# Litianyu141/Gen-FVGN-steady

Hardware: AMD Instinct MI355X
Metric: training iters/sec, 50k-cell cylinder mesh (fwd + loss + bwd + Adam, batch resident in HBM) (higher is better)
Workload: dtype f32

## Files before the change

### gen-fvgn-steady_amd/csrc/colchain.hip

```cpp
#include "colchain_kernel.h"

int* gfv_internal_status_ptr();

static int cc_env(const char* name, int dflt) {
  const char* e = getenv(name);
  return e ? atoi(e) : dflt;
}
static bool al16(const void* p) { return (reinterpret_cast<size_t>(p) & 15) == 0; }

static int cc_cus() {
  static int n = 0;
  if (!n) {
    int dev = 0;
    hipDeviceProp_t pr;
    if (hipGetDevice(&dev) == hipSuccess && hipGetDeviceProperties(&pr, dev) == hipSuccess) n = pr.multiProcessorCount;
    if (n <= 0) n = 256;
    const int want = cc_env("GFV_COLCHAIN_WGS", 0);
    if (want > 0 && want <= n) n = want;
  }
  return n;
}

static bool cc_bwd_ok(const gfv_rowtile_args_t* a) {
  static const int on = cc_env("GFV_COLCHAIN_BWD", 1);
  static const int min_m = cc_env("GFV_COLCHAIN_BWD_MIN_M", 2048);
  if (a->flags & GFV_CHAIN_ROW_OWNER) return false;
  if (!(a->flags & GFV_CHAIN_COLUMN_OWNER) && (!on || a->M < min_m)) return false;
  if (!a->dw_partial || a->dw_partial_stride < GFV_DW_FUSED_FLOATS || !a->in_stats || !a->wmax) return false;
  if (a->dw_in) return false;
  const bool noout = a->nlayers == 2;
  const bool rc = a->rc_Wh[0] != nullptr;
  if (rc && (!a->rc_Wh[1] || a->dw_in || !al16(a->rc_Wh[0]) || !al16(a->rc_Wh[1]) || (a->rc_bias[0] && !al16(a->rc_bias[0])) ||
             (a->rc_bias[1] && !al16(a->rc_bias[1]))))
    return false;
  if (!rc && a->rc_Wh[1]) return false;
  if ((a->nlayers != 3 && !noout) || a->in_op != GFV_IN_LNBWD || a->fin_op != GFV_FIN_PLAIN || a->nseg != 1) return false;
  if (noout && (a->layer[1].op != GFV_OP_MUL_DGELU || a->layer[1].save || a->res[0] || a->gadd || a->dw_in || !a->out[0])) return false;
  if (a->seg[0].width != 128 || a->seg[0].idx || a->seg[0].csr_rowptr || a->seg[0].save || a->seg[0].ld != 128 || !al16(a->seg[0].ptr)) return false;
  if (a->M > (1 << 22) || a->out_ld[0] != 128 || (a->res[0] && a->res_ld[0] != 128) || (a->dw_in && a->dw_in_ld != 128)) return false;
  if (a->layer[0].op != GFV_OP_MUL_DGELU || a->layer[1].op != GFV_OP_MUL_DGELU || (!noout && a->layer[2].op != GFV_OP_NONE)) return false;
  for (int l = 0; l < a->nlayers; ++l) {
    const gfv_layer_t& L = a->layer[l];
    if (!L.Wh || (L.N != 128 && !(l == 2 && L.N == 192)) || L.K != 128 || L.bias || L.bias2) return false;
    if (l < 2 && !(rc && l == 0) && (!L.aux || !al16(L.aux))) return false;
    if (L.save && !al16(L.save)) return false;
  }
  if ((!rc && (!a->in_aux || !al16(a->in_aux))) || !a->in_gamma || !al16(a->in_gamma) || a->ln_partial || a->padd) return false;
  const bool out2 = !noout && a->layer[2].N == 192;
  if (!a->out[0] || (out2 ? (!a->out[1] || a->out_ld[1] != 64 || !al16(a->out[1]) || a->dw_in) : a->out[1] != nullptr) || a->out[2] ||
      a->res[1] || a->res[2] || a->out_nores)
    return false;
  if ((a->out_ld[0] & 3) || !al16(a->out[0]) || (a->res[0] && ((a->res_ld[0] & 3) || !al16(a->res[0])))) return false;
  if (a->in_add && !al16(a->in_add)) return false;
  if (a->gadd && (!al16(a->gadd) || !a->gadd_s || !a->gadd_r)) return false;
  if (a->in_save && !al16(a->in_save)) return false;
  if ((reinterpret_cast<size_t>(a->in_stats) & 7) || !al16(a->dw_partial) || (a->dw_partial_stride & 3)) return false;
  return true;
}
extern "C" int gfv_hidden_size(void);
extern "C" int gfv_f16split_enabled(void);
extern "C" int gfv_rowtile_dw_partials(void) { return cc_cus(); }
extern "C" int gfv_rowtile_dw_partials_m(int32_t M) {
  const int tiles = (M + 63) / 64;
  return tiles < cc_cus() ? (tiles > 0 ? tiles : 1) : cc_cus();
}
extern "C" int gfv_rowtile_fuses_dw(const gfv_rowtile_args_t* a) {
  if (!a || gfv_hidden_size() != 128 || gfv_f16split_enabled() == 0) return 0;
  gfv_rowtile_args_t t = *a;
  t.hidden = 128;
  return cc_bwd_ok(&t) ? 1 : 0;
}

int gfv_internal_colchain_try(const gfv_rowtile_args_t* a, hipStream_t stream) {
  if (a->hidden == 128 && cc_bwd_ok(a)) {
    int* st = gfv_internal_status_ptr();
    if (!st) return 0;
    const dim3 grid(gfv_rowtile_dw_partials_m(a->M)), blk(64 * CC_W);
#define CB_K(...) GFV_LAUNCH((colchain_bwd_kernel<__VA_ARGS__>), grid, blk, 0, stream, *a, st)
#define CB_LAUNCH(LOWP, RC)                                                                                                      \
  do {                                                                                                                           \
    if (a->nlayers == 2) CB_K(LOWP, false, false, true, RC);                                                                     \
    else if (a->layer[2].N == 192 && a->gadd) CB_K(LOWP, true, true, false, RC);                                                 \
    else if (a->layer[2].N == 192) CB_K(LOWP, false, true, false, RC);                                                           \
    else if (a->gadd) CB_K(LOWP, true, false, false, RC);                                                                        \
    else CB_K(LOWP, false, false, false, RC);                                                                                    \
  } while (0)
    const bool rc = a->rc_Wh[0] != nullptr;
    if (a->product_form == 2) { if (rc) CB_LAUNCH(2, true); else CB_LAUNCH(2, false); }
    else if (a->product_form != 0) { if (rc) CB_LAUNCH(1, true); else CB_LAUNCH(1, false); }
    else { if (rc) CB_LAUNCH(0, true); else CB_LAUNCH(0, false); }
#undef CB_K
#undef CB_LAUNCH
    return 2;
  }
  return 0;
}
```

### gen-fvgn-steady_amd/csrc/colchain_kernel.h

```cpp
#pragma once
#include "tchain_kernel.h"

namespace {

constexpr int CC_W = 8;
constexpr float CC_SH = 16.0f;
constexpr float CC_SH_INV = 1.0f / 16.0f;
constexpr float CC_SH_LIMIT = 2048.0f;
#ifdef GFV_CC_TIMING
#define CT_DECL long long ct_[16] = {0, 0, 0, 0, 0, 0, 0, 0, 0, 0, 0, 0, 0, 0, 0, 0}; long long ct_prev_ = clock64();
#define CT(k) do { __builtin_amdgcn_s_waitcnt(0xc07f); const long long now_ = clock64(); ct_[k] += now_ - ct_prev_; ct_prev_ = now_; } while (0)
#else
#define CT_DECL
#define CT(k)
#endif
__device__ __forceinline__ void cc_barrier() {
  asm volatile("s_waitcnt lgkmcnt(0)\n\ts_barrier" ::: "memory");
}

struct CcCtx {
  int w, lane, j, g, col0;
  int M;
  int row0;
  int ngt;
  float invw;
  float mabs;
};

template <int KT, int LOWP, bool FENCE = false>
__device__ __forceinline__ void cc_mma_pair(const char* xbuf, int pair, const gfv_f16x8 (&wh)[KT], const gfv_f16x8 (&wl)[KT],
                                            int lane, floatx4& a0, floatx4& a1) {
  const gfv_f16x8* f0 = reinterpret_cast<const gfv_f16x8*>(xbuf + (size_t)(2 * pair) * KT * 2048) + lane;
  const gfv_f16x8* f1 = f0 + KT * 128;
  a0 = floatx4{0.f, 0.f, 0.f, 0.f};
  a1 = floatx4{0.f, 0.f, 0.f, 0.f};
#pragma unroll
  for (int T = 0; T < KT; ++T) {
    const gfv_f16x8 xh0 = f0[(2 * T) * 64], xh1 = f1[(2 * T) * 64];
    if (!LOWP) {
      const gfv_f16x8 xl0 = f0[(2 * T + 1) * 64], xl1 = f1[(2 * T + 1) * 64];
      a0 = __builtin_amdgcn_mfma_f32_16x16x32_f16(wl[T], xh0, a0, 0, 0, 0);
      a1 = __builtin_amdgcn_mfma_f32_16x16x32_f16(wl[T], xh1, a1, 0, 0, 0);
      a0 = __builtin_amdgcn_mfma_f32_16x16x32_f16(wh[T], xl0, a0, 0, 0, 0);
      a1 = __builtin_amdgcn_mfma_f32_16x16x32_f16(wh[T], xl1, a1, 0, 0, 0);
    }
    a0 = gfv_mma_hh<LOWP == 2>(wh[T], xh0, a0);
    a1 = gfv_mma_hh<LOWP == 2>(wh[T], xh1, a1);
    if (FENCE) __builtin_amdgcn_sched_barrier(0);
  }
}

template <bool BF>
__device__ __forceinline__ void cc_put_frag(char* xbuf, int q, const CcCtx& c, const float (&a)[4], float scale) {
  unsigned h0, h1, l0, l1;
  const gfv_f2 s01 = gfv_f2{a[0], a[1]} * gfv_splat2(scale), s23 = gfv_f2{a[2], a[3]} * gfv_splat2(scale);
  gfv_split_pair_t<BF>(s01.x, s01.y, h0, l0);
  gfv_split_pair_t<BF>(s23.x, s23.y, h1, l1);
  char* dst = xbuf + (size_t)((q * 4 + (c.w >> 1)) * 2) * 1024 + c.lane * 16 + (c.w & 1) * 8;
  *reinterpret_cast<uint2*>(dst) = make_uint2(h0, h1);
  *reinterpret_cast<uint2*>(dst + 1024) = make_uint2(l0, l1);
}

constexpr int CB_TG = 4;
struct CbLds {
  static constexpr int BUF = CB_TG * 8192;
  static constexpr int B0 = 0, B1 = BUF, B2 = 2 * BUF;
  static constexpr int PART = 3 * BUF;
  static constexpr int SMAX = PART + CB_TG * 16 * 8 * 8;
  static constexpr int TOTAL = SMAX + 64;
};

__device__ __forceinline__ void cb_tr_operand(const char* xbuf, int q0, int ct, int lane, gfv_f16x8& hi, gfv_f16x8& lo) {
  typedef short s4 __attribute__((ext_vector_type(4)));
  typedef __attribute__((address_space(3))) s4* lds_s4;
  const int s = lane & 15, gp = lane >> 4;
  const int off = ((q0 * 4 + (ct >> 1)) * 2) * 1024 + (16 * (s & 3) + 4 * gp + (s >> 2)) * 16 + (ct & 1) * 8;
  const char* p = xbuf + off;
  const s4 h0 = __builtin_amdgcn_ds_read_tr16_b64_v4i16((lds_s4)(p));
  const s4 l0 = __builtin_amdgcn_ds_read_tr16_b64_v4i16((lds_s4)(p + 1024));
  const s4 h1 = __builtin_amdgcn_ds_read_tr16_b64_v4i16((lds_s4)(p + 8192));
  const s4 l1 = __builtin_amdgcn_ds_read_tr16_b64_v4i16((lds_s4)(p + 8192 + 1024));
  typedef short s8 __attribute__((ext_vector_type(8)));
  const s8 h = {h0[0], h0[1], h0[2], h0[3], h1[0], h1[1], h1[2], h1[3]};
  const s8 l = {l0[0], l0[1], l0[2], l0[3], l1[0], l1[1], l1[2], l1[3]};
  hi = __builtin_bit_cast(gfv_f16x8, h);
  lo = __builtin_bit_cast(gfv_f16x8, l);
}

__device__ __forceinline__ int cb_dw_ntile(int w, int i) { return 2 * (w >> 1) + (i >> 2); }
__device__ __forceinline__ int cb_dw_ktile(int w, int i) { return 4 * (w & 1) + (i & 3); }
__device__ __forceinline__ int cb_dw_btile(int w) { return 2 * (w >> 1) + (w & 1); }
template <int LOWP>
__device__ __forceinline__ void cb_dw_tile(const char* gbuf, const char* abuf, int npairs, int w, int lane, floatx4 (&acc)[8],
                                           floatx4& accb) {
  const gfv_f16x8 ones = gfv_frag_ones<LOWP == 2>();
  const int nt0 = 2 * (w >> 1), kt0 = 4 * (w & 1);
  for (int pr = 0; pr < npairs; ++pr) {
    gfv_f16x8 gh[2], gl[2];
    cb_tr_operand(gbuf, 2 * pr, nt0, lane, gh[0], gl[0]);
    cb_tr_operand(gbuf, 2 * pr, nt0 + 1, lane, gh[1], gl[1]);
    {
      const bool odd = (w & 1) != 0;
      const gfv_f16x8 bh = odd ? gh[1] : gh[0], bl = odd ? gl[1] : gl[0];
      if (!LOWP) accb = __builtin_amdgcn_mfma_f32_16x16x32_f16(bl, ones, accb, 0, 0, 0);
      accb = gfv_mma_hh<LOWP == 2>(bh, ones, accb);
    }
#pragma unroll
    for (int kk = 0; kk < 4; ++kk) {
      gfv_f16x8 ah, al;
      cb_tr_operand(abuf, 2 * pr, kt0 + kk, lane, ah, al);
#pragma unroll
      for (int nn = 0; nn < 2; ++nn) {
        if (!LOWP) {
          acc[4 * nn + kk] = __builtin_amdgcn_mfma_f32_16x16x32_f16(gl[nn], ah, acc[4 * nn + kk], 0, 0, 0);
          acc[4 * nn + kk] = __builtin_amdgcn_mfma_f32_16x16x32_f16(gh[nn], al, acc[4 * nn + kk], 0, 0, 0);
        }
        acc[4 * nn + kk] = gfv_mma_hh<LOWP == 2>(gh[nn], ah, acc[4 * nn + kk]);
      }
    }
    __builtin_amdgcn_sched_barrier(0);
  }
}

template <bool BF>
__device__ __forceinline__ void cb_hidden_bwd(CcCtx& c, int q, const floatx4& acc, float inv_in, const float4& z, float sg,
                                              char* gout, char* aout, float (&v)[4]) {
  const gfv_f2 z01 = {z.x, z.y}, z23 = {z.z, z.w};
  gfv_f2 a01, a23, d01, d23;
  gfv_gelu_dgelu2(z01, a01, d01);
  gfv_gelu_dgelu2(z23, a23, d23);
  const gfv_f2 ki = gfv_splat2(inv_in), kw = gfv_splat2(c.invw);
  const gfv_f2 v01 = ((gfv_f2{acc[0], acc[1]} * ki) * kw) * d01, v23 = ((gfv_f2{acc[2], acc[3]} * ki) * kw) * d23;
  v[0] = v01.x; v[1] = v01.y; v[2] = v23.x; v[3] = v23.y;
  const float a[4] = {a01.x, a01.y, a23.x, a23.y};
  const float mq = max3_abs(max3_abs(0.f, v[0], v[1]), v[2], v[3]) * sg;
  const float ma = max3_abs(max3_abs(0.f, a[0], a[1]), a[2], a[3]) * (60000.0f / CC_SH_LIMIT);
  c.mabs = fmaxf(c.mabs, q < c.ngt ? fmaxf(mq, ma) : 0.f);
  cc_put_frag<BF>(gout, q, c, v, sg);
  cc_put_frag<BF>(aout, q, c, a, CC_SH);
}

__device__ __forceinline__ char* cb_own_slot(char* xbuf, int q, const CcCtx& c) {
  return xbuf + (size_t)((q * 4 + (c.w >> 1)) * 2) * 1024 + c.lane * 16 + (c.w & 1) * 8;
}
__device__ __forceinline__ void cb_park4(char* xbuf, int q, const CcCtx& c, const float (&v)[4]) {
  char* d = cb_own_slot(xbuf, q, c);
  *reinterpret_cast<float2*>(d) = make_float2(v[0], v[1]);
  *reinterpret_cast<float2*>(d + 1024) = make_float2(v[2], v[3]);
}
__device__ __forceinline__ void cb_unpark4(char* xbuf, int q, const CcCtx& c, float (&v)[4]) {
  const char* d = cb_own_slot(xbuf, q, c);
  const float2 a = *reinterpret_cast<const float2*>(d), b = *reinterpret_cast<const float2*>(d + 1024);
  v[0] = a.x; v[1] = a.y; v[2] = b.x; v[3] = b.y;
}

template <bool BF>
__device__ __forceinline__ void cb_hidden_bwd_dg(CcCtx& c, int q, const floatx4& acc, float inv_in, const float (&dg)[4], float sg,
                                                 char* gout, float (&v)[4]) {
#pragma unroll
  for (int r = 0; r < 4; ++r) v[r] = ((acc[r] * inv_in) * c.invw) * dg[r];
  const float mq = max3_abs(max3_abs(0.f, v[0], v[1]), v[2], v[3]) * sg;
  c.mabs = fmaxf(c.mabs, q < c.ngt ? mq : 0.f);
  cc_put_frag<BF>(gout, q, c, v, sg);
}

typedef int cb_i32x4 __attribute__((ext_vector_type(4)));
typedef int cb_i32x2 __attribute__((ext_vector_type(2)));
typedef __amdgpu_buffer_rsrc_t cb_rsrc;
constexpr int CB_OFF_DEAD = 0x7ffffff0;
__device__ __forceinline__ cb_rsrc cb_buf(const void* p, size_t bytes) {
  const size_t n = p ? (bytes < 0x7fffffe0ull ? bytes : 0x7fffffe0ull) : 0;
  return __builtin_amdgcn_make_buffer_rsrc(const_cast<void*>(p), 0, (int)n, 0x00020000);
}
typedef float cb_f32x2 __attribute__((ext_vector_type(2)));
__device__ __forceinline__ float4 cb_ld4(cb_rsrc r, int off) {
  const floatx4 f = __builtin_bit_cast(floatx4, __builtin_amdgcn_raw_buffer_load_b128(r, off, 0, 0));
  return make_float4(f[0], f[1], f[2], f[3]);
}
__device__ __forceinline__ float2 cb_ld2(cb_rsrc r, int off) {
  const cb_f32x2 f = __builtin_bit_cast(cb_f32x2, __builtin_amdgcn_raw_buffer_load_b64(r, off, 0, 0));
  return make_float2(f[0], f[1]);
}
__device__ __forceinline__ void cb_st4v(cb_rsrc r, int off, const floatx4& f) {
  __builtin_amdgcn_raw_buffer_store_b128(__builtin_bit_cast(cb_i32x4, f), r, off, 0, 0);
}
__device__ __forceinline__ void cb_st4(cb_rsrc r, int off, const float (&v)[4]) {
  const floatx4 f = {v[0], v[1], v[2], v[3]};
  __builtin_amdgcn_raw_buffer_store_b128(__builtin_bit_cast(cb_i32x4, f), r, off, 0, 0);
}

struct CbIn {
  float4 dy[CB_TG], yv[CB_TG], ga[CB_TG];
  float2 st[CB_TG];
};
struct CbBufs {
  cb_rsrc dy, y3, stats, z2, z1, gadd, gidx, save1, res, out;
};
__device__ __forceinline__ int cb_off(const CcCtx& c, int row0, int q) { return min(row0 + 16 * q + c.j, c.M - 1) * 512 + c.col0 * 4; }

template <bool GADD>
__device__ __forceinline__ void cb_load_gidx(const CbBufs& B, const CcCtx& c, int row0, int (&gidx)[CB_TG]) {
  if (GADD) {
#pragma unroll
    for (int q = 0; q < CB_TG; ++q) gidx[q] = __builtin_amdgcn_raw_buffer_load_b32(B.gidx, min(row0 + 16 * q + c.j, c.M - 1) * 4, 0, 0);
  }
}
__device__ __forceinline__ void cb_load_inputs(const CbBufs& B, const CcCtx& c, int row0, CbIn& in) {
#pragma unroll
  for (int q = 0; q < CB_TG; ++q) {
    const int off = cb_off(c, row0, q);
    in.dy[q] = cb_ld4(B.dy, off);
    in.yv[q] = cb_ld4(B.y3, off);
    in.st[q] = cb_ld2(B.stats, min(row0 + 16 * q + c.j, c.M - 1) * 8);
  }
}
__device__ __forceinline__ void cb_load_dy_stats(const CbBufs& B, const CcCtx& c, int row0, CbIn& in) {
#pragma unroll
  for (int q = 0; q < CB_TG; ++q) {
    in.dy[q] = cb_ld4(B.dy, cb_off(c, row0, q));
    in.st[q] = cb_ld2(B.stats, min(row0 + 16 * q + c.j, c.M - 1) * 8);
  }
}
__device__ __forceinline__ void cb_load_rows(cb_rsrc r, const CcCtx& c, int row0, float4 (&v)[CB_TG]) {
#pragma unroll
  for (int q = 0; q < CB_TG; ++q) v[q] = cb_ld4(r, cb_off(c, row0, q));
}
template <bool GADD>
__device__ __forceinline__ void cb_load_gathers(const CbBufs& B, const CcCtx& c, const int (&gidx)[CB_TG], CbIn& in) {
  if (GADD) {
#pragma unroll
    for (int q = 0; q < CB_TG; ++q) in.ga[q] = cb_ld4(B.gadd, gidx[q] * 256 + (c.col0 & 63) * 4);
  }
}

template <int LOWP, bool GADD, bool OUT2 = false, bool NOOUT = false, bool RC = false>
__global__ __launch_bounds__(64 * CC_W, 2) void colchain_bwd_kernel(const gfv_rowtile_args_t A, int* status) {
  constexpr int TG = CB_TG;
  __shared__ __attribute__((aligned(16))) char lds[CbLds::TOTAL + (RC ? CbLds::BUF : 0)];
  char* b0 = lds + CbLds::B0;
  char* b1 = lds + CbLds::B1;
  char* b2 = lds + CbLds::B2;
  char* b3 = lds + CbLds::TOTAL;
  float* part = reinterpret_cast<float*>(lds + CbLds::PART);
  float* smax = reinterpret_cast<float*>(lds + CbLds::SMAX);

  CcCtx c;
  c.w = __builtin_amdgcn_readfirstlane(threadIdx.x >> 6);
  c.lane = threadIdx.x & 63;
  c.j = c.lane & 15;
  c.g = c.lane >> 4;
  c.col0 = 16 * c.w + 4 * c.g;
  c.M = A.M;
  c.mabs = 0.f;
  c.invw = 1.0f / gfv_pow2_scale(*A.wmax);

  const int nwg = gridDim.x;
  const int wg = (nwg & 7) == 0 ? (int)(blockIdx.x & 7) * (nwg >> 3) + (int)(blockIdx.x >> 3) : (int)blockIdx.x;
  const int NG = (A.M + 15) >> 4;
  const int g_beg = (int)((long)NG * wg / nwg), g_end = (int)((long)NG * (wg + 1) / nwg);

  const size_t rows128 = (size_t)A.M * 512;
  CbBufs B;
  B.dy = cb_buf(A.seg[0].ptr, rows128);
  B.y3 = cb_buf(RC ? nullptr : A.in_aux, rows128);
  B.stats = cb_buf(A.in_stats, (size_t)A.M * 8);
  B.z2 = cb_buf(RC ? nullptr : A.layer[0].aux, rows128);
  B.z1 = cb_buf(A.layer[1].aux, rows128);
  B.gadd = cb_buf(A.gadd, 0x7fffffe0ull);
  B.gidx = cb_buf(c.w < 4 ? A.gadd_s : A.gadd_r, (size_t)A.M * 4);
  B.save1 = cb_buf(NOOUT ? A.out[0] : A.layer[1].save, rows128);
  B.res = cb_buf(NOOUT ? nullptr : A.res[0], rows128);
  B.out = cb_buf(NOOUT ? nullptr : A.out[0], rows128);
  const cb_rsrc out2 = cb_buf(OUT2 ? A.out[1] : nullptr, (size_t)A.M * 256);

  const cb_rsrc w0 = cb_buf(A.layer[0].Wh, 65536), w1 = cb_buf(A.layer[1].Wh, 65536),
                w2 = cb_buf(NOOUT ? nullptr : A.layer[2].Wh, OUT2 ? 131072 : 65536);
  const cb_rsrc rw2 = cb_buf(RC ? A.rc_Wh[0] : nullptr, 65536), rw3 = cb_buf(RC ? A.rc_Wh[1] : nullptr, 65536);
  const int woff = (c.w * 128 + c.lane) * 16;
  floatx4 dw3[8], dw2[8], db3 = floatx4{0.f, 0.f, 0.f, 0.f}, db2 = db3;
#pragma unroll
  for (int kt = 0; kt < 8; ++kt) dw3[kt] = dw2[kt] = floatx4{0.f, 0.f, 0.f, 0.f};
  float dgam[4] = {0.f, 0.f, 0.f, 0.f}, dbet[4] = {0.f, 0.f, 0.f, 0.f};
  float sacc = 0.f;
  float scap = 3.0e38f;

  float step1, step2;
  {
    float l1[2];
#pragma unroll
    for (int l = 0; l < 2; ++l) {
      const cb_rsrc wb = l == 0 ? w0 : w1;
      float acc = 0.f;
#pragma unroll
      for (int T = 0; T < 4; ++T) {
        const gfv_f16x8 h = __builtin_bit_cast(gfv_f16x8, __builtin_amdgcn_raw_buffer_load_b128(wb, woff + T * 16384, 0, 0));
        const gfv_f16x8 lo = __builtin_bit_cast(gfv_f16x8, __builtin_amdgcn_raw_buffer_load_b128(wb, woff + T * 16384 + 1024, 0, 0));
        if (LOWP == 2) {
          const gfv_bf16x8 hb = __builtin_bit_cast(gfv_bf16x8, h);
#pragma unroll
          for (int e = 0; e < 8; ++e) acc += fabsf((float)hb[e]);
        } else {
#pragma unroll
          for (int e = 0; e < 8; ++e) acc += fabsf((float)h[e] + (float)lo[e]);
        }
      }
      l1[l] = gfv_wave_max(row_sum(acc));
    }
    if (c.lane == 0) { smax[c.w] = l1[0]; part[c.w] = l1[1]; }
    cc_barrier();
    float m0 = 0.f, m1 = 0.f;
#pragma unroll
    for (int k = 0; k < 8; ++k) { m0 = fmaxf(m0, smax[k]); m1 = fmaxf(m1, part[k]); }
    cc_barrier();
    const float g0 = 1.13f * m0 * c.invw, g1 = 1.13f * m1 * c.invw;
    step1 = 1.0f / gfv_pow2_ceil(g0);
    step2 = 1.0f / gfv_pow2_ceil(g1);
  }

  constexpr bool PRE = true;
  int gidx[TG] = {0, 0, 0, 0};
  CbIn in;
  float4 zn[RC ? TG : 1];
  if (g_beg < g_end) {
    cb_load_gidx<GADD>(B, c, 16 * g_beg, gidx);
    if constexpr (RC) {
      cb_load_rows(B.z1, c, 16 * g_beg, zn);
      cb_load_dy_stats(B, c, 16 * g_beg, in);
      cb_load_gathers<GADD>(B, c, gidx, in);
    } else if (PRE) {
      cb_load_inputs(B, c, 16 * g_beg, in);
      cb_load_gathers<GADD>(B, c, gidx, in);
    }
  }
  const bool CB_LATE = c.w >= 4;
  CT_DECL
  for (int t0 = g_beg; t0 < g_end; t0 += TG) {
    c.row0 = 16 * t0;
    c.ngt = min(TG, g_end - t0);
    const int np = (c.ngt + 1) >> 1;
    const int next_row0 = t0 + TG < g_end ? 16 * (t0 + TG) : c.M;
    int offL[TG], offS[TG];
#pragma unroll
    for (int q = 0; q < TG; ++q) {
      const int row = c.row0 + 16 * q + c.j;
      offL[q] = cb_off(c, c.row0, q);
      offS[q] = (q < c.ngt && row < c.M) ? row * 512 + c.col0 * 4 : CB_OFF_DEAD;
    }
    if constexpr (RC) {
      gfv_f16x8 rh[4], rl[4];
#pragma unroll
      for (int T = 0; T < 4; ++T) {
        rh[T] = __builtin_bit_cast(gfv_f16x8, __builtin_amdgcn_raw_buffer_load_b128(rw2, woff + T * 16384, 0, 0));
        rl[T] = __builtin_bit_cast(gfv_f16x8, __builtin_amdgcn_raw_buffer_load_b128(rw2, woff + T * 16384 + 1024, 0, 0));
      }
      const float4 zero4 = make_float4(0.f, 0.f, 0.f, 0.f);
#pragma unroll
      for (int q = 0; q < TG; ++q) {
        const float z4[4] = {zn[q].x, zn[q].y, zn[q].z, zn[q].w};
        float a[4];
#pragma unroll
        for (int r = 0; r < 4; ++r) a[r] = gfv_gelu(z4[r]);
        const float ma = max3_abs(max3_abs(0.f, a[0], a[1]), a[2], a[3]) * (60000.0f / CC_SH_LIMIT);
        c.mabs = fmaxf(c.mabs, q < c.ngt ? ma : 0.f);
        cc_put_frag<LOWP == 2>(b3, q, c, a, CC_SH);
      }
      CT(12);
      cc_barrier();
      CT(13);
#pragma unroll
      for (int q = 0; q < TG; ++q) in.yv[q] = zero4;
      {
        int tvar = 0;
        asm volatile("" : "+v"(tvar));
        const float4 bi2 = cb_ld4(cb_buf(A.rc_bias[0], 512), c.col0 * 4 + tvar);
        floatx4 a0, a1;
        cc_mma_pair<4, LOWP, true>(b3, 0, rh, rl, c.lane, a0, a1);
#pragma unroll
        for (int p = 0; p < TG / 2; ++p) {
          if (p >= np) break;
          floatx4 n0 = a0, n1 = a1;
          if (p + 1 < TG / 2) cc_mma_pair<4, LOWP, true>(b3, p + 1, rh, rl, c.lane, n0, n1);
#pragma unroll
          for (int h = 0; h < 2; ++h) {
            const int q = 2 * p + h;
            const floatx4& acc = h ? a1 : a0;
            const float bb[4] = {bi2.x, bi2.y, bi2.z, bi2.w};
            float a[4], dg[4];
#pragma unroll
            for (int r = 0; r < 4; ++r) {
              const float z = (acc[r] * CC_SH_INV) * c.invw + bb[r];
              const gfv_erfc_t e = gfv_erfc_half(z);
              const float cdf = z >= 0.0f ? 1.0f - e.y : e.y;
              dg[r] = fmaf(z * 0.39894228040143267794f, e.e, cdf);
              a[r] = fmaf(-fabsf(z), e.y, fmaxf(z, 0.0f));
            }
            cb_park4(b1, q, c, dg);
            const float ma = max3_abs(max3_abs(0.f, a[0], a[1]), a[2], a[3]) * (60000.0f / CC_SH_LIMIT);
            c.mabs = fmaxf(c.mabs, q < c.ngt ? ma : 0.f);
            cc_put_frag<LOWP == 2>(b2, q, c, a, CC_SH);
          }
          a0 = n0; a1 = n1;
        }
      }
#pragma unroll
      for (int T = 0; T < 4; ++T) {
        rh[T] = __builtin_bit_cast(gfv_f16x8, __builtin_amdgcn_raw_buffer_load_b128(rw3, woff + T * 16384, 0, 0));
        rl[T] = __builtin_bit_cast(gfv_f16x8, __builtin_amdgcn_raw_buffer_load_b128(rw3, woff + T * 16384 + 1024, 0, 0));
      }
      CT(14);
      cc_barrier();
      CT(15);
      {
        int tvar = 0;
        asm volatile("" : "+v"(tvar));
        const float4 bi3 = cb_ld4(cb_buf(A.rc_bias[1], 512), c.col0 * 4 + tvar);
        floatx4 a0, a1;
        cc_mma_pair<4, LOWP, true>(b2, 0, rh, rl, c.lane, a0, a1);
#pragma unroll
        for (int p = 0; p < TG / 2; ++p) {
          if (p >= np) break;
          floatx4 n0 = a0, n1 = a1;
          if (p + 1 < TG / 2) cc_mma_pair<4, LOWP, true>(b2, p + 1, rh, rl, c.lane, n0, n1);
          in.yv[2 * p] = make_float4((a0[0] * CC_SH_INV) * c.invw + bi3.x, (a0[1] * CC_SH_INV) * c.invw + bi3.y,
                                     (a0[2] * CC_SH_INV) * c.invw + bi3.z, (a0[3] * CC_SH_INV) * c.invw + bi3.w);
          in.yv[2 * p + 1] = make_float4((a1[0] * CC_SH_INV) * c.invw + bi3.x, (a1[1] * CC_SH_INV) * c.invw + bi3.y,
                                         (a1[2] * CC_SH_INV) * c.invw + bi3.z, (a1[3] * CC_SH_INV) * c.invw + bi3.w);
          a0 = n0; a1 = n1;
        }
      }
    }
    float gg[TG][4], xh[TG][4], rs[TG];
    {
      float bmax = 0.f;
      if (!PRE) {
        cb_load_inputs(B, c, c.row0, in);
        cb_load_gathers<GADD>(B, c, gidx, in);
      }
      if (A.in_add) {
        const cb_rsrc ia = cb_buf(A.in_add, rows128);
#pragma unroll
        for (int q = 0; q < TG; ++q) {
          const float4 t = cb_ld4(ia, offL[q]);
          in.dy[q].x += t.x; in.dy[q].y += t.y; in.dy[q].z += t.z; in.dy[q].w += t.w;
        }
      }
      float* part_j = part + (c.j * 8 + c.w) * 2;
      const float4 gam = RC ? cb_ld4(cb_buf(A.in_gamma, 512), c.col0 * 4) : ld4(A.in_gamma + c.col0);
#pragma unroll
      for (int q = 0; q < TG; ++q) {
        const float lf = offS[q] != CB_OFF_DEAD ? 1.0f : 0.0f;
        float d[4] = {in.dy[q].x, in.dy[q].y, in.dy[q].z, in.dy[q].w};
        if (GADD) { d[0] += in.ga[q].x; d[1] += in.ga[q].y; d[2] += in.ga[q].z; d[3] += in.ga[q].w; }
        const float y[4] = {in.yv[q].x, in.yv[q].y, in.yv[q].z, in.yv[q].w};
        const float gm[4] = {gam.x, gam.y, gam.z, gam.w};
        const float mean = in.st[q].x, rstd = in.st[q].y;
        rs[q] = rstd;
        float s1 = 0.f, s2 = 0.f, am = 0.f;
#pragma unroll
        for (int h = 0; h < 2; ++h) {
          const int r = 2 * h;
          const gfv_f2 dd = gfv_f2{d[r], d[r + 1]} * gfv_splat2(lf);
          const gfv_f2 xx = (gfv_f2{y[r], y[r + 1]} - gfv_splat2(mean)) * gfv_splat2(rstd);
          const gfv_f2 dx = dd * xx;
          const gfv_f2 g2 = dd * gfv_f2{gm[r], gm[r + 1]};
          const gfv_f2 gx = g2 * xx;
          const gfv_f2 ng = gfv_f2{dgam[r], dgam[r + 1]} + dx, nb = gfv_f2{dbet[r], dbet[r + 1]} + dd;
          dgam[r] = ng.x; dgam[r + 1] = ng.y;
          dbet[r] = nb.x; dbet[r + 1] = nb.y;
          xh[q][r] = xx.x; xh[q][r + 1] = xx.y;
          gg[q][r] = g2.x; gg[q][r + 1] = g2.y;
          s1 += g2.x; s1 += g2.y;
          s2 += gx.x; s2 += gx.y;
          am = max3_abs(am, g2.x, g2.y);
        }
        s1 = row_sum(s1);
        s2 = row_sum(s2);
        if (c.g == 0) *reinterpret_cast<float2*>(part_j + q * 256) = make_float2(s1, s2);
        bmax = fmaxf(bmax, am * fabsf(rstd) * lf);
      }
      bmax = gfv_wave_max(bmax);
      if (c.lane == 0) smax[c.w] = bmax;
    }
    gfv_f16x8 wh[4], wl[4];
#pragma unroll
    for (int T = 0; T < 4; ++T) {
      wh[T] = __builtin_bit_cast(gfv_f16x8, __builtin_amdgcn_raw_buffer_load_b128(w0, woff + T * 16384, 0, 0));
      wl[T] = __builtin_bit_cast(gfv_f16x8, __builtin_amdgcn_raw_buffer_load_b128(w0, woff + T * 16384 + 1024, 0, 0));
    }
    float4 zq[TG];
    if constexpr (!RC) {
#pragma unroll
      for (int q = 0; q < TG; ++q) zq[q] = cb_ld4(B.z2, offL[q]);
    }
    CT(0);
    cc_barrier();
    CT(1);
    float s3;
    {
      const float4 ma = *reinterpret_cast<const float4*>(smax), mb = *reinterpret_cast<const float4*>(smax + 4);
      const float mx = fmaxf(fmaxf(fmaxf(ma.x, ma.y), fmaxf(ma.z, ma.w)), fmaxf(fmaxf(mb.x, mb.y), fmaxf(mb.z, mb.w)));
      s3 = fminf(gfv_pow2_scale(mx * 13.5f) * 2.0f, scap);
      scap = fminf(scap, s3 * 1048576.0f);
#pragma unroll
      for (int q = 0; q < TG; ++q) {
        const float4* pp = reinterpret_cast<const float4*>(part + (q * 16 + c.j) * 16);
        const float4 p0 = pp[0], p1 = pp[1], p2 = pp[2], p3 = pp[3];
        const float m1 = (((p0.x + p0.z) + (p1.x + p1.z)) + ((p2.x + p2.z) + (p3.x + p3.z))) * 0.0078125f;
        const float m2 = (((p0.y + p0.w) + (p1.y + p1.w)) + ((p2.y + p2.w) + (p3.y + p3.w))) * 0.0078125f;
        float g3[4];
#pragma unroll
        for (int h = 0; h < 2; ++h) {
          const int r = 2 * h;
          const gfv_f2 t = gfv_splat2(rs[q]) * ((gfv_f2{gg[q][r], gg[q][r + 1]} - gfv_splat2(m1)) - gfv_f2{xh[q][r], xh[q][r + 1]} * gfv_splat2(m2));
          g3[r] = t.x; g3[r + 1] = t.y;
        }
        if (A.in_save) cb_st4(cb_buf(A.in_save, rows128), offS[q], g3);
        cc_put_frag<LOWP == 2>(b0, q, c, g3, s3);
      }
    }
    if (sacc != 0.f && sacc != s3) {
      const float ratio = s3 / sacc;
#pragma unroll
      for (int kt = 0; kt < 8; ++kt) { dw3[kt] *= ratio; dw2[kt] *= ratio; }
      db3 *= ratio;
      db2 *= ratio;
    }
    sacc = s3;
    const float s2s = s3 * step1, s1s = s2s * step2;
    if (A.gscale && c.w == 0 && c.lane < c.ngt) {
      const size_t grp = (size_t)(c.row0 >> 4) + c.lane;
      A.gscale[grp] = s3 * 0.25f;
      A.gscale[(size_t)A.gscale_ld + grp] = s2s * 0.25f;
      A.gscale[2 * (size_t)A.gscale_ld + grp] = s1s * 0.25f;
    }
    CT(2);
    cc_barrier();
    CT(3);
    cb_load_gidx<GADD>(B, c, next_row0, gidx);
    {
      const float inv_in = 1.0f / s3;
      floatx4 a0, a1;
      cc_mma_pair<4, LOWP, true>(b0, 0, wh, wl, c.lane, a0, a1);
#pragma unroll
      for (int p = 0; p < TG / 2; ++p) {
        if (p >= np) break;
        floatx4 n0 = a0, n1 = a1;
        float v0[4], v1[4];
        if (!CB_LATE && p + 1 < TG / 2) cc_mma_pair<4, LOWP, true>(b0, p + 1, wh, wl, c.lane, n0, n1);
        if constexpr (RC) {
          float d0[4], d1[4];
          cb_unpark4(b1, 2 * p, c, d0);
          cb_unpark4(b1, 2 * p + 1, c, d1);
          cb_hidden_bwd_dg<LOWP == 2>(c, 2 * p, a0, inv_in, d0, s2s, b1, v0);
          cb_hidden_bwd_dg<LOWP == 2>(c, 2 * p + 1, a1, inv_in, d1, s2s, b1, v1);
        } else {
          cb_hidden_bwd<LOWP == 2>(c, 2 * p, a0, inv_in, zq[2 * p], s2s, b1, b2, v0);
          cb_hidden_bwd<LOWP == 2>(c, 2 * p + 1, a1, inv_in, zq[2 * p + 1], s2s, b1, b2, v1);
        }
        if (A.layer[0].save) {
          const cb_rsrc s0 = cb_buf(A.layer[0].save, rows128);
          cb_st4(s0, offS[2 * p], v0);
          cb_st4(s0, offS[2 * p + 1], v1);
        }
        if (CB_LATE && p + 1 < TG / 2) cc_mma_pair<4, LOWP, true>(b0, p + 1, wh, wl, c.lane, n0, n1);
        a0 = n0; a1 = n1;
      }
    }
#pragma unroll
    for (int T = 0; T < 4; ++T) {
      wh[T] = __builtin_bit_cast(gfv_f16x8, __builtin_amdgcn_raw_buffer_load_b128(w1, woff + T * 16384, 0, 0));
      wl[T] = __builtin_bit_cast(gfv_f16x8, __builtin_amdgcn_raw_buffer_load_b128(w1, woff + T * 16384 + 1024, 0, 0));
    }
#pragma unroll
    for (int q = 0; q < TG; ++q) zq[q] = cb_ld4(B.z1, offL[q]);
    CT(4);
    cc_barrier();
    CT(5);
    if constexpr (RC) cb_load_rows(B.z1, c, next_row0, zn);
    cb_dw_tile<LOWP>(b0, b2, np, c.w, c.lane, dw3, db3);
    if constexpr (RC) cb_dw_tile<LOWP>(b1, b3, np, c.w, c.lane, dw2, db2);
    CT(6);
    cc_barrier();
    CT(7);
    {
      const float inv_in = 1.0f / s2s;
      floatx4 a0, a1;
      cc_mma_pair<4, LOWP, true>(b1, 0, wh, wl, c.lane, a0, a1);
#pragma unroll
      for (int p = 0; p < TG / 2; ++p) {
        if (p >= np) break;
        floatx4 n0 = a0, n1 = a1;
        float v0[4], v1[4];
        if (!CB_LATE && p + 1 < TG / 2) cc_mma_pair<4, LOWP, true>(b1, p + 1, wh, wl, c.lane, n0, n1);
        if constexpr (RC) {
          const float d0[4] = {gfv_dgelu(zq[2 * p].x), gfv_dgelu(zq[2 * p].y), gfv_dgelu(zq[2 * p].z), gfv_dgelu(zq[2 * p].w)};
          const float d1[4] = {gfv_dgelu(zq[2 * p + 1].x), gfv_dgelu(zq[2 * p + 1].y), gfv_dgelu(zq[2 * p + 1].z),
                               gfv_dgelu(zq[2 * p + 1].w)};
          cb_hidden_bwd_dg<LOWP == 2>(c, 2 * p, a0, inv_in, d0, s1s, b0, v0);
          cb_hidden_bwd_dg<LOWP == 2>(c, 2 * p + 1, a1, inv_in, d1, s1s, b0, v1);
        } else {
          cb_hidden_bwd<LOWP == 2>(c, 2 * p, a0, inv_in, zq[2 * p], s1s, b0, b2, v0);
          cb_hidden_bwd<LOWP == 2>(c, 2 * p + 1, a1, inv_in, zq[2 * p + 1], s1s, b0, b2, v1);
        }
        cb_st4(B.save1, offS[2 * p], v0);
        cb_st4(B.save1, offS[2 * p + 1], v1);
        if (CB_LATE && p + 1 < TG / 2) cc_mma_pair<4, LOWP, true>(b1, p + 1, wh, wl, c.lane, n0, n1);
        a0 = n0; a1 = n1;
      }
    }
    if constexpr (!NOOUT) {
#pragma unroll
      for (int T = 0; T < 4; ++T) {
        wh[T] = __builtin_bit_cast(gfv_f16x8, __builtin_amdgcn_raw_buffer_load_b128(w2, woff + T * 16384, 0, 0));
        wl[T] = __builtin_bit_cast(gfv_f16x8, __builtin_amdgcn_raw_buffer_load_b128(w2, woff + T * 16384 + 1024, 0, 0));
      }
    }
    float4 rr[NOOUT ? 1 : TG];
    if constexpr (!NOOUT) {
#pragma unroll
      for (int q = 0; q < TG; ++q) rr[q] = cb_ld4(B.res, offL[q]);
    }
    CT(8);
    cc_barrier();
    CT(9);
    if constexpr (!NOOUT) {
      const float inv_in = 1.0f / s1s;
      floatx4 a0, a1;
      cc_mma_pair<4, LOWP, true>(b0, 0, wh, wl, c.lane, a0, a1);
#pragma unroll
      for (int p = 0; p < TG / 2; ++p) {
        if (p >= np) break;
        floatx4 n0 = a0, n1 = a1;
        if (!CB_LATE && p + 1 < TG / 2) cc_mma_pair<4, LOWP, true>(b0, p + 1, wh, wl, c.lane, n0, n1);
        const floatx4 o0 = (a0 * inv_in) * c.invw + floatx4{rr[2 * p].x, rr[2 * p].y, rr[2 * p].z, rr[2 * p].w};
        const floatx4 o1 = (a1 * inv_in) * c.invw + floatx4{rr[2 * p + 1].x, rr[2 * p + 1].y, rr[2 * p + 1].z, rr[2 * p + 1].w};
        cb_st4v(B.out, offS[2 * p], o0);
        cb_st4v(B.out, offS[2 * p + 1], o1);
        if (CB_LATE && p + 1 < TG / 2) cc_mma_pair<4, LOWP, true>(b0, p + 1, wh, wl, c.lane, n0, n1);
        a0 = n0; a1 = n1;
      }
      if constexpr (OUT2) {
        if (c.w < 4) {
          gfv_f16x8 xh2[4], xl2[4];
#pragma unroll
          for (int T = 0; T < 4; ++T) {
            xh2[T] = __builtin_bit_cast(gfv_f16x8, __builtin_amdgcn_raw_buffer_load_b128(w2, 65536 + woff + T * 16384, 0, 0));
            xl2[T] = __builtin_bit_cast(gfv_f16x8, __builtin_amdgcn_raw_buffer_load_b128(w2, 65536 + woff + T * 16384 + 1024, 0, 0));
          }
#pragma unroll
          for (int p = 0; p < TG / 2; ++p) {
            if (p >= np) break;
            floatx4 e0, e1;
            cc_mma_pair<4, LOWP, true>(b0, p, xh2, xl2, c.lane, e0, e1);
            const floatx4 o0 = (e0 * inv_in) * c.invw, o1 = (e1 * inv_in) * c.invw;
            const int ra = c.row0 + 32 * p + c.j, rb = ra + 16;
            cb_st4v(out2, (2 * p < c.ngt && ra < c.M) ? ra * 256 + c.col0 * 4 : CB_OFF_DEAD, o0);
            cb_st4v(out2, (2 * p + 1 < c.ngt && rb < c.M) ? rb * 256 + c.col0 * 4 : CB_OFF_DEAD, o1);
          }
        }
      }
    }
    CT(10);
    if constexpr (RC) {
      cb_load_dy_stats(B, c, next_row0, in);
      cb_load_gathers<GADD>(B, c, gidx, in);
    } else {
      if (PRE) {
        cb_load_inputs(B, c, next_row0, in);
        cb_load_gathers<GADD>(B, c, gidx, in);
      }
      cb_dw_tile<LOWP>(b1, b2, np, c.w, c.lane, dw2, db2);
    }
    CT(11);
  }

#ifdef GFV_CC_TIMING
  if (c.lane == 0 && A.fin_aux) {
    long long* dbg = reinterpret_cast<long long*>(const_cast<float*>(A.fin_aux)) + ((size_t)blockIdx.x * CC_W + c.w) * 16;
    for (int kk = 0; kk < 16; ++kk) dbg[kk] = ct_[kk];
  }
#endif
  if (A.dw_partial) {
    float* blk = A.dw_partial + (size_t)blockIdx.x * A.dw_partial_stride;
    const float is = sacc != 0.f ? 1.0f / sacc : 0.f;
    const float r2 = 1.0f / step1, r1 = r2 / step2;
    const float u3 = is * CC_SH_INV, u2 = (is * r2) * CC_SH_INV;
#pragma unroll
    for (int kt = 0; kt < 8; ++kt)
#pragma unroll
      for (int r = 0; r < 4; ++r) {
        const int n = 16 * cb_dw_ntile(c.w, kt) + 4 * c.g + r, k = 16 * cb_dw_ktile(c.w, kt) + c.j;
        blk[n * 128 + k] = dw3[kt][r] * u3;
        blk[16384 + 128 + n * 128 + k] = dw2[kt][r] * u2;
      }
    if (c.j == 0) {
#pragma unroll
      for (int r = 0; r < 4; ++r) {
        const int nb = 16 * cb_dw_btile(c.w) + 4 * c.g + r;
        blk[16384 + nb] = db3[r] * is;
        blk[2 * 16384 + 128 + nb] = db2[r] * (is * r2);
      }
    }
#pragma unroll
    for (int r = 0; r < 4; ++r) {
      const float dg = gfv_row16_sum(dgam[r]), db = gfv_row16_sum(dbet[r]);
      if (c.j == 0) {
        blk[2 * 16384 + 256 + c.col0 + r] = dg;
        blk[2 * 16384 + 384 + c.col0 + r] = db;
      }
    }
  }
  if (c.mabs > 60000.0f) atomicOr(status, 2);
}


}
```

### gen-fvgn-steady_amd/csrc/rowtile.hip

```cpp
#include <atomic>
#include <stdio.h>
#include <stdlib.h>
#include <mutex>
#include "gfv_common.h"
#include "gfv_limits.h"
#include "gfv_prof.h"
#include "../../include/gfv.h"

namespace {
constexpr int BM = 64;
}

int gfv_internal_tchain_launch(const gfv_rowtile_args_t* args, int ragged, int f16, hipStream_t stream);

static std::atomic<int> g_f16_default{-1};
static thread_local int g_f16split = -1;
static int f16_default() {
  int d = g_f16_default.load(std::memory_order_relaxed);
  if (d < 0) {
    const char* e = getenv("GFV_F16SPLIT");
    d = e ? ((atoi(e) == 2 || atoi(e) == 3) ? atoi(e) : (atoi(e) != 0)) : 1;
    int expect = -1;
    if (!g_f16_default.compare_exchange_strong(expect, d)) d = expect;
  }
// ... 40 lines not shown
}
}
int gfv_internal_limit(int which) {
  std::call_once(g_limit_once, limits_init);
  return (which >= 0 && which < GFV_LIM_COUNT) ? g_limit[which] : 0;
}
extern "C" int gfv_get_limit(int32_t which) { return (which >= 0 && which < GFV_LIM_COUNT) ? gfv_internal_limit(which) : -1; }
extern "C" int gfv_set_limit(int32_t which, int32_t value) {
  if (which < 0 || which >= GFV_LIM_COUNT) return GFV_ERR_ARG;
  std::call_once(g_limit_once, limits_init);
  if (value < 0) {
    const char* e = getenv(k_limits[which].env);
    g_limit[which] = e ? atoi(e) : k_limits[which].dflt;
  } else {
    g_limit[which] = value;
  }
  return GFV_OK;
}
extern "C" const char* gfv_limit_name(int32_t which) { return (which >= 0 && which < GFV_LIM_COUNT) ? k_limits[which].env : nullptr; }

static thread_local int g_last_ln_rows = 0;
extern "C" int gfv_rowtile_last_ln_rows(void) { return g_last_ln_rows; }

extern "C" int gfv_rowtile_tiles(int32_t M) { return (M + BM - 1) / BM; }

static int rowtile_chain_impl(const gfv_rowtile_args_t* args, void* stream);
extern "C" int gfv_rowtile_chain(const gfv_rowtile_args_t* args, void* stream) {
  if (!args) return GFV_ERR_ARG;
  if (args->product_form < 0 || args->product_form > 4 || (args->hidden != 0 && (args->hidden < 16 || args->hidden > 128 || (args->hidden & 15))))
    return GFV_ERR_ARG;
  if (args->product_form == 0 && args->hidden == 0) return rowtile_chain_impl(args, stream);
  const int f0 = g_f16split, h0 = g_hidden;
  if (args->product_form) g_f16split = args->product_form - 1;
  if (args->hidden) g_hidden = args->hidden;
  const int rc = rowtile_chain_impl(args, stream);
  g_f16split = f0;
  g_hidden = h0;
  return rc;
}
int gfv_internal_lin1_try(const gfv_rowtile_args_t* a, int lowp, hipStream_t stream, int dry);
int gfv_internal_cfwd_try(const gfv_rowtile_args_t* a, int lowp, hipStream_t stream, int dry);
bool gfv_internal_wimg_form_ok(const float* wmax);
int gfv_internal_cbwd_try(const gfv_rowtile_args_t* a, int lowp, hipStream_t stream, int dry);
static int cfwd_try(const gfv_rowtile_args_t* args, int lowp, hipStream_t stream, int dry) {
  if (args->nlayers != 3 || (args->fin_op != GFV_FIN_LN && args->fin_op != GFV_FIN_PLAIN)) return 0;
  gfv_rowtile_args_t local = *args;
  local.hidden = g_hidden;
  return gfv_internal_cfwd_try(&local, lowp, stream, dry);
}
static int cbwd_try(const gfv_rowtile_args_t* args, int lowp, hipStream_t stream, int dry) {
  if (args->in_op != GFV_IN_LNBWD || args->dw_partial || !args->in_stats) return 0;
  gfv_rowtile_args_t local = *args;
  local.hidden = g_hidden;
  return gfv_internal_cbwd_try(&local, lowp, stream, dry);
}
static int rowtile_chain_impl(const gfv_rowtile_args_t* args, void* stream) {
  if (!args || args->M < 0 || args->nlayers < 1 || args->nlayers > 3 || args->nseg < 1 || args->nseg > 3) return GFV_ERR_ARG;
  if (args->M == 0) {
    g_last_ln_rows = 0;
    return GFV_OK;
  }
  for (int i = 0; i < args->nseg; ++i)
    if (args->seg[i].width < 1 || args->seg[i].width > 128) return GFV_ERR_ARG;
  for (int l = 0; l + 1 < args->nlayers; ++l)
    if (args->layer[l].N != 128 || args->layer[l + 1].K != 128) return GFV_ERR_ARG;
  int k0 = 0;
  for (int i = 0; i < args->nseg; ++i) k0 += args->seg[i].width;
  if (k0 != args->layer[0].K) return GFV_ERR_ARG;
  const gfv_layer_t& last = args->layer[args->nlayers - 1];
  if (last.N > 384 || last.N < 1) return GFV_ERR_ARG;
  if ((args->rc_Wh[0] || args->rc_Wh[1]) && !args->dw_partial) return GFV_ERR_ARG;
  if (args->padd && (args->nlayers < 2 || args->padd_ld < 256 || (args->padd_ld & 3) || !args->padd_s || !args->padd_r)) return GFV_ERR_ARG;
  for (int l = 0; l < args->nlayers; ++l)
    if (args->layer[l].ldw != 0 && args->layer[l].ldw < args->layer[l].K) return GFV_ERR_ARG;
  if (last.N > 128 && (last.N & 15)) return GFV_ERR_ARG;
  if ((args->fin_op != GFV_FIN_PLAIN || args->in_op == GFV_IN_LN || args->in_op == GFV_IN_LNBWD) &&
      (args->fin_op != GFV_FIN_PLAIN ? last.N != 128 : false))
    return GFV_ERR_ARG;
  if ((args->in_op == GFV_IN_LN || args->in_op == GFV_IN_LNBWD) && (args->nseg != 1 || args->seg[0].width != 128))
    return GFV_ERR_ARG;
  bool fast_t = true;
  for (int i = 0; i < args->nseg; ++i) fast_t = fast_t && (args->seg[i].width % 32 == 0) && (args->seg[i].ld % 4 == 0);
  for (int l = 0; l < args->nlayers; ++l) {
    const bool lastl = (l == args->nlayers - 1);
    fast_t = fast_t && (args->layer[l].K % 4 == 0) && (args->layer[l].ldw % 4 == 0) && (args->layer[l].N % (lastl ? 64 : 128) == 0);
  }
  if (args->fin_op != GFV_FIN_PLAIN) fast_t = fast_t && last.N == 128;
  for (int c = 0; c < 3; ++c) {
    if (args->out[c]) fast_t = fast_t && (args->out_ld[c] % 4 == 0);
    if (args->res[c]) fast_t = fast_t && (args->res_ld[c] % 4 == 0);
  }
  bool rag_t = !fast_t && args->in_op != GFV_IN_LNBWD && args->fin_op != GFV_FIN_LNBWD;
  for (int l = 0; l + 1 < args->nlayers; ++l) rag_t = rag_t && args->layer[l].N == 128;
  if (last.N > 128) rag_t = rag_t && (last.N % 64 == 0);
  if (last.N % 16) rag_t = rag_t && last.op != GFV_OP_MUL_DGELU && args->fin_op == GFV_FIN_PLAIN && !args->out_nores;
  if (args->in_op == GFV_IN_LN) rag_t = rag_t && args->seg[0].width == 128 && (args->seg[0].ld % 4 == 0);
  if (args->gadd) rag_t = rag_t && args->seg[0].width == 128 && (args->seg[0].ld % 4 == 0);
  for (int l = 1; l < args->nlayers; ++l) rag_t = rag_t && (args->layer[l].K == 128);
  {
    bool csr = false;
    for (int i = 0; i < args->nseg; ++i) {
      const gfv_seg_t& sg = args->seg[i];
      csr = csr || sg.csr_rowptr != nullptr || sg.save != nullptr;
      if (sg.csr_rowptr && (!sg.idx || (i == 0 && args->in_add))) return GFV_ERR_ARG;
    }
    if (csr && (!fast_t || args->in_op == GFV_IN_LNBWD || args->fin_op == GFV_FIN_LNBWD))
      return GFV_ERR_ARG;
  }
  bool f16 = (fast_t || rag_t) && f16_mode() != 0 && args->wmax != nullptr;
  for (int l = 0; l < args->nlayers; ++l) f16 = f16 && args->layer[l].Wh != nullptr;
  for (int i = 0; i + 1 < args->nseg; ++i) f16 = f16 && (args->seg[i].width % 32 == 0);
  if (f16 && !gfv_internal_wimg_form_ok(args->wmax)) return GFV_ERR_ARG;
  for (int l = 0; l < args->nlayers; ++l)
    if ((!args->layer[l].W || args->layer[l].bias2) && !f16) return GFV_ERR_ARG;
  if (!fast_t && !rag_t) {
    static const bool dbg = getenv("GFV_ROWTILE_DEBUG") != nullptr;
    if (dbg)
      fprintf(stderr, "[gfv] gfv_rowtile_chain: unsupported shape M=%d nseg=%d widths=%d,%d,%d ld0=%d nlayers=%d K0=%d Nlast=%d out_ld=%d in_op=%d fin_op=%d\n",
              args->M, args->nseg, args->seg[0].width, args->nseg > 1 ? args->seg[1].width : 0,
              args->nseg > 2 ? args->seg[2].width : 0, args->seg[0].ld, args->nlayers, args->layer[0].K, last.N,
              args->out_ld[0], args->in_op, args->fin_op);
    return GFV_ERR_ARG;
  }
  void* tok = nullptr;
  if (gfv_prof_enabled()) {
    double fl = 0, by = 0;
    for (int l = 0; l < args->nlayers; ++l) {
      fl += 2.0 * args->M * (double)args->layer[l].K * args->layer[l].N;
      by += 4.0 * ((double)args->layer[l].K * args->layer[l].N + args->layer[l].N);
      if (args->layer[l].save) by += 4.0 * args->M * args->layer[l].N;
      if (args->layer[l].aux) by += 4.0 * args->M * args->layer[l].N;
    }
    by += 4.0 * args->M * (double)args->layer[0].K + 4.0 * args->M * (double)last.N;
    for (int i = 0; i < args->nseg; ++i) if (args->seg[i].idx) by += 4.0 * args->M;
    if (args->in_aux || args->fin_aux) by += 4.0 * args->M * 128.0;
    if (args->in_save) by += 4.0 * args->M * 128.0;
    if (args->fin_presave) by += 4.0 * args->M * 128.0;
    if (args->out_nores) by += 4.0 * args->M * 128.0;
    if (args->padd) by += 4.0 * args->M * 258.0;
    for (int c = 0; c < 3; ++c) if (args->res[c]) by += 4.0 * args->M * 128.0;
    const int lnm = args->in_op == GFV_IN_LNBWD ? 1 : (args->fin_op == GFV_FIN_LNBWD ? 2 : 0);
    int kind = fast_t ? GFV_K_TCHAIN0 + lnm : GFV_K_TCHAIN_RAG;
    for (int i = 0; i < args->nseg; ++i)
      if (args->seg[i].csr_rowptr || args->seg[i].save) kind = GFV_K_TCHAIN_CSR;
    if (fast_t && f16 && args->nlayers == 1 && gfv_internal_lin1_try(args, f16_mode() >= 2 ? f16_mode() - 1 : 0, (hipStream_t)stream, 1))
      kind = GFV_K_LIN1;
    if (f16 && cfwd_try(args, f16_mode() >= 2 ? f16_mode() - 1 : 0, (hipStream_t)stream, 1))
      kind = GFV_K_COLCHAIN_FWD;
    if (args->dw_partial) {
      kind = GFV_K_COLCHAIN_BWD;
      const int nfused = 2 + (args->rc_Wh[0] ? 2 : 0);
      fl += nfused * 2.0 * args->M * 128.0 * 128.0;
      by += 8.0 * args->M + 4.0 * (double)gfv_rowtile_dw_partials_m(args->M) * (double)args->dw_partial_stride;
    }
    tok = gfv_prof_begin(kind, fl, by, (hipStream_t)stream);
  }
  g_last_path = (fast_t ? 1 : 2) + (f16 ? 4 : 0);
  g_last_ln_rows = (args->M + BM - 1) / BM;
  if (args->dw_partial && !(fast_t && f16)) return GFV_ERR_ARG;
  if (fast_t && f16 && args->nlayers == 1 && gfv_internal_lin1_try(args, f16_mode() >= 2 ? f16_mode() - 1 : 0, (hipStream_t)stream, 0)) {
    g_last_path += 32;
  } else if (f16 && !args->dw_partial && cfwd_try(args, f16_mode() >= 2 ? f16_mode() - 1 : 0, (hipStream_t)stream, 0)) {
    g_last_path += 64;
  } else if (fast_t && f16 && cbwd_try(args, f16_mode() >= 2 ? f16_mode() - 1 : 0, (hipStream_t)stream, 0)) {
    g_last_path += 128;
    g_last_ln_rows = (args->M + 31) / 32;
  } else if (fast_t) {
    const int took = gfv_internal_tchain_launch(args, 0, f16 ? 1 : 0, (hipStream_t)stream);
    if (args->dw_partial && took != 2) return GFV_ERR_ARG;
    g_last_path += 8 * took;
  }
  else
    gfv_internal_tchain_launch(args, 1, f16 ? 1 : 0, (hipStream_t)stream);
  gfv_prof_end(tok, (hipStream_t)stream);
  GFV_CHECK_LAUNCH();
  return GFV_OK;
}
```

### gen-fvgn-steady_amd/gfv/engine.py

```python
from __future__ import annotations

import contextlib
import os
import struct

import torch

from . import cmdlist
from . import lib as L
from . import ops
from .ops import LayerSpec, Seg

_MODE = {"explicit": 0, "implicit": 1, "imex": 2}


def _empty(dev, *shape):
    return torch.empty(shape, dtype=torch.float32, device=dev)


def pick_concurrent_stream(priority=0, candidates=8):
    if torch.cuda.is_current_stream_capturing():
        return torch.cuda.Stream(priority=priority)
    main = torch.cuda.current_stream()
    cycles = 400_000

    def timed(side):
        torch.cuda.synchronize()
        e0, e1 = torch.cuda.Event(enable_timing=True), torch.cuda.Event(enable_timing=True)
        e0.record(main)
        if side is not None:
            side.wait_stream(main)
            with torch.cuda.stream(side):
                torch.cuda._sleep(cycles)
        torch.cuda._sleep(cycles)
        if side is not None:
            main.wait_stream(side)
        e1.record(main)
        torch.cuda.synchronize()
        return e0.elapsed_time(e1)

    timed(None)
    alone = min(timed(None) for _ in range(2))
    first = None
    for _ in range(candidates):
        cand = torch.cuda.Stream(priority=priority)
        first = first or cand
        timed(cand)
        if min(timed(cand) for _ in range(2)) < 1.5 * alone:
            return cand
    return first


class GradStore:

    def __init__(self, names, shapes, device, flat=None, skip=()):
        self.off, self.shape = {}, {}
        off = 0
        for n, sh in zip(names, shapes):
            k = 1
            for d in sh:
                k *= int(d)
            self.off[n], self.shape[n] = off, tuple(sh)
            off += (k + 3) // 4 * 4
        self.total = off
        self.flat = torch.zeros(off, dtype=torch.float32, device=device) if flat is None else flat
        self.skip = set(skip)

    def numel(self, n):
        k = 1
        for d in self.shape[n]:
            k *= d
        return k

    def view(self, n):
        if n in self.skip:
            return None
        return self.flat[self.off[n]:self.off[n] + self.numel(n)].view(self.shape[n])

    def view_of(self, buf, n):
        return buf[self.off[n]:self.off[n] + self.numel(n)].view(self.shape[n])

    def block(self, first, last):
        end = self.off[last] + (self.numel(last) + 3) // 4 * 4
        return self.off[first], end - self.off[first]


class Engine:
    def __init__(self, message_passing_num=3, integrator="imex", ncn_smooth=True, net="TransFVGN_v2", conserved_form=True,
                 order="2nd", hidden=128):
        self.hidden = int(hidden)
        self._dw_ws, self._dw_ws_main = None, None
        self._pending = []
        self._defer_mode = os.environ.get("GFV_DEFER", "1") == "1"
        self._wt, self._wt_key, self._wt_live = {}, None, False
        self._wt_desc, self._wt_n, self._wt_max = None, 0, (0, 0)
        self._last_gn = False
        self.mp = message_passing_num
        self.mode = _MODE[integrator]
        self.smooth = 1 if ncn_smooth else 0
        self.nc = 0 if conserved_form else 1
        if order not in ("1st", "2nd", "3rd", "4th"):
            raise ValueError("order must be specified in [\"1st\", \"2nd\", \"3rd\", \"4th\"]")
        self.order_terms = {"1st": 2, "2nd": 5, "3rd": 9, "4th": 14}[order]
        self.n_proc = 2 if net in ("TransFVGN_v2", "TransFVGN") else 1
        self.net = net
        self.overlap = os.environ.get("GFV_OVERLAP", "1") != "0"
        self.factor = os.environ.get("GFV_EDGE_FACTOR", "1") != "0"
        self.f16split = os.environ.get("GFV_F16SPLIT", "1") != "0"
        self.csr_fuse = ops.csr_prologue_enabled()
        self._fuse_mask = int(os.environ.get("GFV_CSR_FUSE_MASK", "4"))
        self._csr1_max = int(os.environ.get("GFV_CSR1_MAX_M", "16384"))
        self.fuse_dw = os.environ.get("GFV_FUSE_DW", "1") != "0"
        self.recompute = os.environ.get("GFV_RECOMPUTE", "0") != "0"
        self._slice_fuse = os.environ.get("GFV_SLICE_FUSE", "1") != "0"
        self._trans_fuse = os.environ.get("GFV_TRANS_FUSE", "1") != "0"
        self._trans_fuse_min = int(os.environ.get("GFV_TRANS_FUSE_MIN_M", "16385"))
        self._trans_fuse_fwd_small = bool(L.get_limit("GFV_CTRANS")) if torch.cuda.is_available() else True
        self._trans_reduce_merge = os.environ.get("GFV_TRANS_REDUCE_MERGE", "1") != "0"
        self._tail_env = ("GFV_TAIL_MAIN" in os.environ) or ("GFV_TAIL_SPLIT" in os.environ)
        self._tail_main = int(os.environ.get("GFV_TAIL_MAIN", "2"))
        self._tail_split = int(os.environ.get("GFV_TAIL_SPLIT", "1"))
        self._fuse_noout = os.environ.get("GFV_FUSE_NOOUT", "1") != "0"
        self._fuse_dw_min = int(os.environ.get("GFV_COLCHAIN_BWD_MIN_M", "2048"))
        self._cbwd_max_fixed = None
        self._wi, self._wi_key, self._wmax, self._wi_abs = None, None, None, None
        self._pkey_cache = None
        self._zero_e = None
        self._etmp = None
        self._prep_ws = None
        self._fvm_cnt = None
        self._fvm_fuse = os.environ.get("GFV_FVM_FUSE", "1") != "0"
        self._agg_ln = os.environ.get("GFV_AGG_LN", "1") != "0"
        self._side, self._sides = None, []
        self._keep = []
        self.dist_world, self.dist_group, self.dist_force = 1, None, False
        self._retired = []
        self.bucket_hook = None

    class _Fork:
        def __init__(self, eng, keep):
            self.eng, self.keep = eng, keep

        def __enter__(self):
            e = self.eng
            if not e.overlap:
                return self
            if e._side is None:
                e._side = pick_concurrent_stream()
                e._sides = [e._side]
            L.stream_wait(e._side, torch.cuda.current_stream())
            e._keep.extend(t for t in self.keep if t is not None)
            self._ctx = torch.cuda.stream(e._side)
            self._ctx.__enter__()
            return self

        def __exit__(self, *exc):
            if self.eng.overlap:
                self._ctx.__exit__(*exc)
            return False

    def fork(self, *keep):
        return Engine._Fork(self, keep)

    @contextlib.contextmanager
    def model_width(self):
        lib = L.load()
        if self.hidden == 128 and lib.gfv_hidden_size() == 128:
            yield
            return
        L.check(lib.gfv_set_hidden_size(self.hidden), "gfv_set_hidden_size")
        try:
            yield
        finally:
            L.check(lib.gfv_set_hidden_size(128), "gfv_set_hidden_size")

    @property
    def _cbwd_max(self):
        if self._cbwd_max_fixed is not None:
            return self._cbwd_max_fixed
        return L.get_limit("GFV_CBWD_MAX_M") if L.get_limit("GFV_CBWD") else 0

    def _tail_cfg(self, pl):
        if self._tail_env:
            return self._tail_main, self._tail_split
        if pl.E < 32000:
            return 2, 0
        return (2, 2) if pl.E < 150000 else (2, 1)

    def defer(self, fn, *keep):
        if not self.overlap:
            fn()
        elif self._defer_mode:
            self._pending.append((fn, keep))
        else:
            with self.fork(*keep):
                fn()

    def flush(self, on_main=False, split=0):
        if not self._pending:
            return
        pend, self._pending = self._pending, []
        if split and len(pend) > 1:
            k = 1 if split == 1 else len(pend) - 1
            main_part, side_part = (pend[:k], pend[k:]) if split == 1 else (pend[k:], pend[:k])
            self._pending = side_part
            self.flush()
            self._pending = main_part
            self.flush(on_main=True)
            return
        if on_main:
            ws, self._dw_ws = self._dw_ws, self._dw_ws_main
            try:
                for fn, _ in pend:
                    fn()
            finally:
                self._dw_ws_main, self._dw_ws = self._dw_ws, ws
            return
        with self.fork(*[t for _, keep in pend for t in keep]):
            for fn, _ in pend:
                fn()

    def join(self):
        self.flush()
        if self.overlap and self._side is not None:
            for sd in self._sides:
                L.stream_wait(torch.cuda.current_stream(), sd)
        self._keep.clear()

    def _pkey(self, P, fresh=False):
        hit = self._pkey_cache
        if fresh or hit is None or hit[0] is not P:
            self._pkey_cache = hit = (P, tuple(t.data_ptr() for t in P.values()))
        return hit[1]

    def _wi_enter(self, phase, P):
        if not self.f16split:
            return None
        key = self._pkey(P, fresh=(phase == "fwd"))
        if self._wi_key != key:
            dev = next(iter(P.values())).device
            self._retired.append((self._wi, self._wmax, self._wi_abs))
            self._wmax = torch.zeros((1,), dtype=torch.float32, device=dev)
            self._wi = {ph: ops.WeightImages(dev, self._wmax) for ph in ("fwd", "bwd")}
            self._wi["fwd"].add_static(P.values())
            mats = [t for t in P.values() if t.dim() == 2 and t.stride(1) == 1]
            self._wi_abs = ops.WeightImages._upload([((t.data_ptr(), t.stride(0), t.shape[0], t.shape[1]), t) for t in mats], dev)
            self._wi_key = key
        wi = self._wi[phase]
        if phase == "fwd":
            L.check(L.load().gfv_weight_absmax(self._wi_abs[0].data_ptr(), self._wi_abs[1], self._wmax.data_ptr(),
                                               L.stream_ptr()), "gfv_weight_absmax")
        elif not wi.static and self._wt:
            wi.add_static(self._wt.values())
            if self.recompute:
                wi.add_static(P.values())
        wi.build()
        return ops.set_weight_images(wi)

    def build_static_images(self, P):
        if not self.f16split:
            return
        prev = self._wi_enter("fwd", P)
        ops.set_weight_images(prev)

    def _wi_static_enter(self, P):
        if not self.f16split:
            return None
        if self._wi is None or self._wi_key != self._pkey(P, fresh=True):
            raise RuntimeError("static weight images belong to another parameter set: call build_static_images(P) first")
        wi = self._wi["fwd"]
        if len(wi.valid) != len(wi.images) and cmdlist.active() is None:
            L.check(L.load().gfv_weight_absmax(self._wi_abs[0].data_ptr(), self._wi_abs[1], self._wmax.data_ptr(),
                                               L.stream_ptr()), "gfv_weight_absmax")
            wi.build()
        return ops.set_weight_images(wi)

    def capture_signature(self):
        wi = self._wi or {}
        return (self._wi_key, self._wt_key, L.load().gfv_f16split_enabled(),
                tuple((ph, len(w.images), None if w._desc is None else w._desc.data_ptr()) for ph, w in sorted(wi.items())))

    def _wi_exit(self, phase, prev):
        if not self.f16split:
            return
        self._wi[phase].invalidate()
        ops.set_weight_images(prev)

    def _T(self, W, perm=False):
        hit = self._wt.get((W.data_ptr(), perm)) if self._wt_live else None
        if hit is not None:
            return hit
        if not perm:
            return ops.transpose(W)
        if perm == "c":
            return ops.transpose(W, col0=256, ncols=128)
        if perm == "ab":
            return torch.cat((ops.transpose(W, col0=0, ncols=128), ops.transpose(W, col0=128, ncols=128)), 1).contiguous()
        out = _empty(W.device, 192, 128)
        ops.transpose(W, out=out[0:128], col0=64, ncols=128)
        ops.transpose(W, out=out[128:192], col0=0, ncols=64)
        return out

    def prepare_transposes(self, P):
        lib = L.load()
        key = self._pkey(P)
        if self._wt_key != key:
            rows = []
            self._retired.append((self._wt, self._wt_desc))
            self._wt = {}
            dev = next(iter(P.values())).device
            for n, W in P.items():
                if not n.endswith(".weight") or W.dim() != 2:
                    continue
                if any(t in n for t in (".to_q.", ".to_k.", ".to_v.", ".in_project_slice.")):
                    continue
                if ".encoder." in n and n.endswith(".0.0.weight"):
                    continue
                r, c = W.shape
                if ".nb_module.net.0.0.weight" in n:
                    out = _empty(dev, 192, 128)
                    rows.append((W.data_ptr() + 4 * 64, out.data_ptr(), r, 128, c, 0))
                    rows.append((W.data_ptr(), out.data_ptr() + 4 * 128 * 128, r, 64, c, 0))
                    self._wt[(W.data_ptr(), True)] = out
                elif self.factor and ".eb_module.net.0.0.weight" in n:
                    oc, oab = _empty(dev, 128, 128), _empty(dev, 128, 256)
                    rows.append((W.data_ptr() + 4 * 256, oc.data_ptr(), r, 128, c, 0))
                    rows.append((W.data_ptr(), oab.data_ptr(), r, 128, c, 256))
                    rows.append((W.data_ptr() + 4 * 128, oab.data_ptr() + 4 * 128, r, 128, c, 256))
                    self._wt[(W.data_ptr(), "c")] = oc
                    self._wt[(W.data_ptr(), "ab")] = oab
                else:
                    out = _empty(dev, c, r)
                    rows.append((W.data_ptr(), out.data_ptr(), r, c, c, 0))
                    self._wt[(W.data_ptr(), False)] = out
            blob = b"".join(struct.pack("<QQiiii", a, b, r, c, ld, ldo) for a, b, r, c, ld, ldo in rows)
            self._wt_desc = torch.frombuffer(bytearray(blob), dtype=torch.uint8).to(dev)
            self._wt_n = len(rows)
            self._wt_max = (max(r[2] for r in rows), max(r[3] for r in rows))
            self._wt_key = key
        L.check(lib.gfv_transpose_batch(self._wt_desc.data_ptr(), self._wt_n, self._wt_max[0], self._wt_max[1],
                                        L.stream_ptr()), "gfv_transpose_batch")
        self._wt_live = True

    @staticmethod
    def _mlp_names(prefix, ln):
        lin = prefix + ".0" if ln else prefix
        return [f"{lin}.0.weight", f"{lin}.0.bias", f"{lin}.2.weight", f"{lin}.2.bias", f"{lin}.4.weight",
                f"{lin}.4.bias"] + ([f"{prefix}.1.weight", f"{prefix}.1.bias"] if ln else [])

    def mlp3_fwd(self, P, prefix, M, segs, *, ln=True, res=None, in_add=None, want_nores=False, keep=True, w1=None,
                 padd=None, saved_segs=None, nores_from_saved=False):
        names = self._mlp_names(prefix, ln)
        W1, b1, W2, b2, W3, b3 = (P[n] for n in names[:6])
        if w1 is not None:
            W1 = w1
        dev = W1.device
        nout = W3.shape[0]
        would_fuse = (ln and self.fuse_dw and self.f16split and self.hidden == 128 and nout == 128
                      and M >= self._fuse_dw_min and M > self._cbwd_max
                      and (self._fuse_noout or all(sg.width % 32 == 0 for sg in segs)))
        fused_bwd = keep and would_fuse
        would_stats = would_fuse or (ln and self.f16split and nout == 128 and M <= self._cbwd_max)
        lean = fused_bwd and self.recompute
        if keep:
            stats = _empty(dev, M, 2) if would_stats else None
            z1 = _empty(dev, M, 128)
            z2 = _empty(dev, M, 128) if not lean else None
            y3 = _empty(dev, M, 128) if (ln and not lean) else None
        else:
            from_saved = (want_nores and nores_from_saved and would_stats and ln and nout == 128
                          and not (would_fuse and self.recompute))
            z1 = z2 = None
            y3 = _empty(dev, M, 128) if from_saved else None
            stats = _empty(dev, M, 2) if from_saved else None
        out = _empty(dev, M, nout)
        if want_nores and nores_from_saved and y3 is not None and stats is not None and nout == 128:
            want_nores = False
        nores = _empty(dev, M, 128) if want_nores else None
        ops.rowtile_chain(
            M, segs,
            [LayerSpec(W1, b1, L.OP_BIAS_GELU, save=z1), LayerSpec(W2, b2, L.OP_BIAS_GELU, save=z2), LayerSpec(W3, b3)],
            [out], in_add=in_add, fin_op=L.FIN_LN if ln else L.FIN_PLAIN,
            fin_gamma=P[names[6]] if ln else None, fin_beta=P[names[7]] if ln else None, fin_presave=y3,
            res=[res] if res is not None else None, out_nores=nores, fin_stats=stats,
            **(dict(padd=padd[0], padd_s=padd[1], padd_r=padd[2]) if padd is not None else {}))
        if not keep:
            return out, nores, dict(y3=y3, stats=stats)
        saved = dict(z1=z1, z2=z2, y3=y3, segs=segs if saved_segs is None else saved_segs, in_add=in_add, M=M, ln=ln,
                     prefix=prefix, stats=stats, lean=lean, fused=fused_bwd)
        return out, nores, saved

    def _rematerialize(self, P, sv):
        if not sv.get("lean") or sv["z2"] is not None:
            return
        names = self._mlp_names(sv["prefix"], sv["ln"])
        M, dev = sv["M"], sv["z1"].device
        sv["z2"], sv["y3"] = _empty(dev, M, 128), _empty(dev, M, 128)
        ops.rowtile_chain(M, [Seg(sv["z1"])], [LayerSpec(P[names[2]], P[names[3]], L.OP_BIAS_GELU, save=sv["z2"]),
                                              LayerSpec(P[names[4]], P[names[5]])], [sv["y3"]], in_op=L.IN_GELU)

    def mlp3_bwd(self, P, sv, G, grads, *, outs=None, res=None, gadd=None, W1t=None, g_ld=None, g_add=None):
        prefix, M, ln = sv["prefix"], sv["M"], sv["ln"]
        names = self._mlp_names(prefix, ln)
        W1, W2, W3 = P[names[0]], P[names[2]], P[names[4]]
        dev = W1.device
        nout = W3.shape[0]
        W3t, W2t = self._T(W3), self._T(W2)
        if (self.fuse_dw and ln and sv.get("fused", sv.get("stats") is not None) and G.stride(0) == 128 and g_ld is None and gadd is None
                and (outs is not None or (res is None and self._fuse_noout))
                and self._mlp3_bwd_fused(P, sv, G, grads, names, W3t, W2t,
                                         None if outs is None else (W1t if W1t is not None else self._T(W1)), outs, res, g_add)):
            return
        self._rematerialize(P, sv)
        gz2, gz1 = _empty(dev, M, 128), _empty(dev, M, 128)
        part = _empty(dev, ops.ln_rows(M), 2, 128) if ln else None
        g3 = _empty(dev, M, 128) if ln else G
        gseg = Seg(G, width=nout, ld=G.stride(0) if g_ld is None else g_ld)
        kw = dict(in_op=L.IN_LNBWD, in_gamma=P[names[6]], in_aux=sv["y3"], in_save=g3, ln_partial=part,
                  in_stats=sv.get("stats")) if ln else {}
        if gadd is not None:
            kw.update(gadd=gadd[0], gadd_s=gadd[1], gadd_r=gadd[2])
        if g_add is not None:
            assert ln, "the addend is folded into the LayerNorm-backward prologue"
            kw.update(in_add=g_add)
        gs = _empty(dev, 3, ops.gscale_ld(M))
        if outs is not None:
            if W1t is None:
                W1t = self._T(W1)
            have = ops.rowtile_chain(M, [gseg],
                                     [LayerSpec(W3t, None, L.OP_MUL_DGELU, save=gz2, aux=sv["z2"]),
                                      LayerSpec(W2t, None, L.OP_MUL_DGELU, save=gz1, aux=sv["z1"]), LayerSpec(W1t)],
                                     outs, res=res, gscale=gs, **kw)
        else:
            have = ops.rowtile_chain(M, [gseg],
                                     [LayerSpec(W3t, None, L.OP_MUL_DGELU, save=gz2, aux=sv["z2"]),
                                      LayerSpec(W2t, None, L.OP_MUL_DGELU, aux=sv["z1"])], [gz1], gscale=gs, **kw)
        tiles_n = ops.last_ln_rows()
        s0, s1, s2 = (gs[0], gs[1], gs[2]) if have else (None, None, None)
        if not ln and (gadd is not None or g_add is not None):
            s0 = None
        tiles = self._first_layer_tiles(sv, gz1, s2)
        tiles.append(self._tile(gz2, 128, Seg(sv["z1"]), a_op=1, gscale=s1))
        tiles.append(self._tile(g3, nout, Seg(sv["z2"]), a_op=1, ldg=(G.stride(0) if g_ld is None else g_ld) if not ln else None,
                                gscale=s0))
        def side():
            lay = [(names[0], names[1], len(sv["segs"])), (names[2], names[3], 1), (names[4], names[5], 1)]
            pieces = [self._slab_piece(grads, lay, self._dw_block(grads, lay, tiles, M, reduce=False))]
            if ln:
                pieces.append(self._ln_piece(part, tiles_n, grads, names[6], names[7]))
            ops.reduce_multi(pieces)
        self.defer(side, gz1, gz2, g3, G, part, gs, sv["z1"], sv["z2"], sv["in_add"], *[sg.t for sg in sv["segs"]],
                   *[sg.idx for sg in sv["segs"]])

    def _mlp3_bwd_fused(self, P, sv, G, grads, names, W3t, W2t, W1t, outs, res, g_add):
        M = sv["M"]
        dev = G.device
        lib = L.load()
        nwg = lib.gfv_rowtile_dw_partials_m(M)
        dwp = _empty(dev, nwg, L.DW_FUSED_FLOATS)
        gz1 = _empty(dev, M, 128)
        gs = _empty(dev, 3, ops.gscale_ld(M))
        if outs is None:
            layers = [LayerSpec(W3t, None, L.OP_MUL_DGELU, aux=sv["z2"]), LayerSpec(W2t, None, L.OP_MUL_DGELU, aux=sv["z1"])]
            outs = [gz1]
        else:
            layers = [LayerSpec(W3t, None, L.OP_MUL_DGELU, aux=sv["z2"]),
                      LayerSpec(W2t, None, L.OP_MUL_DGELU, save=gz1, aux=sv["z1"]), LayerSpec(W1t)]
        kw = dict(res=res, in_op=L.IN_LNBWD, in_gamma=P[names[6]], in_aux=sv["y3"], in_stats=sv["stats"], dw_partial=dwp, gscale=gs,
                  in_add=g_add, rc=(P[names[2]], P[names[3]], P[names[4]], P[names[5]]) if sv["z2"] is None else None)
        if not ops.rowtile_chain(M, [Seg(G)], layers, outs, query_fused=True, **kw):
            return False
        ops.rowtile_chain(M, [Seg(G)], layers, outs, **kw)
        segs = sv["segs"]
        fused_pieces = self._fused_pieces(dwp, nwg, grads, names)

        def side():
            lay = [(names[0], names[1], len(segs))]
            first = self._dw_block(grads, lay, self._first_layer_tiles(sv, gz1, gs[2]), M, reduce=False)
            ops.reduce_multi([self._slab_piece(grads, lay, first)] + fused_pieces)
        self.defer(side, dwp, gz1, gs, sv["in_add"], *[sg.t for sg in segs], *[sg.idx for sg in segs])
        return True

    @staticmethod
    def _gview2(grads, n0, n1):
        off, length = grads.block(n0, n1)
        return grads.flat[off:off + length]

    @staticmethod
    def _piece(partial, out, n_chunks, chunk_stride, cols, rows=1, ld_out=None):
        p = dict(partial=partial, out=out, n_chunks=n_chunks, chunk_stride=chunk_stride, rows=rows, cols=cols)
        if ld_out is not None:
            p["ld_out"] = ld_out
        return p

    def _ln_piece(self, part, n_rows, grads, gamma, beta):
        return self._piece(part, self._gview2(grads, gamma, beta), n_rows, 256, 256)

    def _fused_pieces(self, dwp, nwg, grads, names):
        base, FL, WB = dwp.data_ptr(), L.DW_FUSED_FLOATS, L.DW_FUSED_WB
        return [self._piece(base + 4 * L.DW_FUSED_OFF_W2, self._gview2(grads, names[2], names[3]), nwg, FL, WB),
                self._piece(base + 4 * L.DW_FUSED_OFF_W3, self._gview2(grads, names[4], names[5]), nwg, FL, WB),
                self._piece(base + 4 * L.DW_FUSED_OFF_LN, self._gview2(grads, names[6], names[7]), nwg, FL, 256)]

    @staticmethod
    def _layers_block(grads, layers):
        last = layers[-1]
        return grads.block(layers[0][0], last[1] if last[1] is not None else last[0])

    def _slab_piece(self, grads, layers, slabs):
        wptr, n, blen, _ = slabs
        return self._piece(wptr, grads.flat.data_ptr() + 4 * self._layers_block(grads, layers)[0], n, blen, blen)

    def _first_layer_tiles(self, sv, gz1, scale):
        return [self._tile(gz1, 128, sg, in_add=sv["in_add"] if i == 0 else None, gscale=scale,
                           a_op=L.DW_COLSCALE if sg.width <= 16 else 0) for i, sg in enumerate(sv["segs"])]

    @staticmethod
    def _tile(G, n_out, seg, *, a_op=0, a_gamma=None, a_beta=None, in_add=None, ldg=None, g_offset=0, gscale=None):
        return dict(G=G, n_out=n_out, seg=seg, a_op=a_op, a_gamma=a_gamma, a_beta=a_beta, in_add=in_add,
                    ldg=G.stride(0) if ldg is None else ldg, g_offset=g_offset, gscale=gscale)

    def _workspace(self, n_floats, dev):
        if self._dw_ws is None or self._dw_ws.numel() < n_floats or self._dw_ws.device != dev:
            self._dw_ws = torch.zeros(int(n_floats * 1.25) + 1024, dtype=torch.float32, device=dev)
        return self._dw_ws

    def _dw_block(self, grads, layers, tiles, M, row0s=None, reduce=True, ws_offset=0):
        lib = L.load()
        off0, blen = self._layers_block(grads, layers)
        ct = (L.DwTile * 6)()
        ti = 0
        for li, (wname, bname, nt) in enumerate(layers):
            K = grads.shape[wname][1]
            koff = 0
            for j in range(nt):
                t, c = tiles[ti], ct[ti]
                sg = t["seg"]
                row0 = 0 if row0s is None else row0s[ti]
                c.G = t["G"].data_ptr() + 4 * t["g_offset"]
                c.A = sg.t.data_ptr() + 4 * sg.offset
                c.idx = None if sg.idx is None else sg.idx.data_ptr()
                c.in_add = None if t["in_add"] is None else t["in_add"].data_ptr()
                c.a_gamma = None if t["a_gamma"] is None else t["a_gamma"].data_ptr()
                c.a_beta = None if t["a_beta"] is None else t["a_beta"].data_ptr()
                c.gscale = None if t.get("gscale") is None else t["gscale"].data_ptr()
                c.ldg, c.n_out, c.width, c.ld = t["ldg"], t["n_out"], sg.width, sg.ld
                c.a_op, c.ld_out = t["a_op"], K
                if row0s is None:
                    c.out_off = grads.off[wname] - off0 + koff
                    c.db_off = (grads.off[bname] - off0) if (bname is not None and j == 0) else -1
                    koff += sg.width
                else:
                    c.out_off = grads.off[wname] - off0 + row0 * K
                    c.db_off = (grads.off[bname] - off0 + row0) if bname is not None else -1
                ti += 1
        need = lib.gfv_dw_multi_workspace_floats(M, ti, blen)
        dev = grads.flat.device
        ws = self._workspace(ws_offset + need, dev)
        wptr = ws.data_ptr() + 4 * ws_offset
        L.check(lib.gfv_dw_multi(ct, ti, M, blen, wptr, (grads.flat.data_ptr() + 4 * off0) if reduce else None, 0,
                                 L.stream_ptr()), "gfv_dw_multi")
        if not reduce:
            return wptr, lib.gfv_dw_slabs(M, ti, None), blen, (need + 3) // 4 * 4

    def _dw_jobs(self, grads, jobs, pieces=()):
        lib = L.load()
        dev = grads.flat.device
        needs = [(lib.gfv_dw_multi_workspace_floats(j["M"], len(j["tiles"]), self._layers_block(grads, j["layers"])[1]) + 3) // 4 * 4
                 for j in jobs]
        self._workspace(sum(needs) + 8, dev)
        out, off = [], 0
        for j, need in zip(jobs, needs):
            slabs = self._dw_block(grads, j["layers"], j["tiles"], j["M"], row0s=j.get("row0s"), reduce=False, ws_offset=off)
            assert slabs[3] <= need
            out.append(self._slab_piece(grads, j["layers"], slabs))
            off += need
        out += list(pieces)
        for k in range(0, len(out), 12):
            ops.reduce_multi(out[k:k + 12])

    @staticmethod
    def _put(grads, name, value):
        cmdlist.call(grads.view(name).copy_, value.reshape(grads.shape[name]))

    def gn_fwd(self, P, prefix, x, e, pl, keep=True):
        N, E = pl.N, pl.E
        fuse = self.csr_fuse
        if self.factor:
            W1 = P[f"{prefix}.eb_module.net.0.0.weight"]
            pab = _empty(x.device, N, 256)
            if fuse and ((self._fuse_mask & 1) or N <= self._csr1_max) and ops.stack_ready(W1[:, 0:128], W1[:, 128:256], rows=True):
                nb = _empty(x.device, N, 128) if keep else None
                ops.rowtile_chain(N, [Seg(x, csr=(pl.n_rowptr, pl.n_col_node), save=nb)],
                                  [LayerSpec(W1[:, 0:128], stack=W1[:, 128:256])], [(pab, 256), (pab.data_ptr() + 512, 256)])
            else:
                nb = ops.seg_gather_sum(x, pl.n_rowptr, pl.n_col_node, N)
                ops.rowtile_chain(N, [Seg(nb)], [LayerSpec(W1[:, 0:128], stack=W1[:, 128:256])],
                                  [(pab, 256), (pab.data_ptr() + 512, 256)])
            e_out, e_new, sv_e = self.mlp3_fwd(P, f"{prefix}.eb_module.net", E, [Seg(e)], res=e, want_nores=True,
                                               w1=W1[:, 256:384], padd=(pab, pl.es, pl.er), nores_from_saved=self._agg_ln, keep=keep)
            sv_e["nb"] = nb
        else:
            nb = ops.seg_gather_sum(x, pl.n_rowptr, pl.n_col_node, N)
            e_out, e_new, sv_e = self.mlp3_fwd(P, f"{prefix}.eb_module.net", E, [Seg(nb, pl.es), Seg(nb, pl.er), Seg(e)],
                                               res=e, want_nores=True, nores_from_saved=self._agg_ln, keep=keep)
        if e_new is None:
            ln_names = self._mlp_names(f"{prefix}.eb_module.net", True)
            agg = ops.seg_gather_sum_ln(sv_e["y3"], sv_e["stats"], P[ln_names[6]], P[ln_names[7]], pl.n_rowptr, pl.n_col_edge2, N)
        else:
            agg = ops.seg_gather_sum(e_new.view(2 * E, 64), pl.n_rowptr, pl.n_col_edge2, N)
        if fuse and (self._fuse_mask & 2):
            nbm = _empty(x.device, N, 128) if keep else None
            x_out, _, sv_n = self.mlp3_fwd(P, f"{prefix}.nb_module.net", N,
                                           [Seg(agg, csr=(pl.n_rowptr, pl.n_col_node), scale=pl.inv_deg, save=nbm), Seg(x)],
                                           res=x, saved_segs=[Seg(nbm, width=64, ld=128), Seg(x)] if keep else None, keep=keep)
        else:
            nbm = ops.seg_gather_sum(agg, pl.n_rowptr, pl.n_col_node, N, scale=pl.inv_deg)
            x_out, _, sv_n = self.mlp3_fwd(P, f"{prefix}.nb_module.net", N, [Seg(nbm), Seg(x)], res=x, keep=keep)
        if not keep:
            return x_out, e_out, None
        return x_out, e_out, dict(sv_e=sv_e, sv_n=sv_n, prefix=prefix)

    def _edge_tmp(self, dev):
        if self._etmp is None or self._etmp[0].flat.device != dev:
            e = GradStore(["W1c", "b1", "W2", "b2", "W3", "b3"], [(128, 128), (128,), (128, 128), (128,), (128, 128), (128,)], dev)
            n = GradStore(["W1ab"], [(128, 256)], dev)
            self._etmp = (e, n)
        return self._etmp

    def _edge_gather_adjoint(self, gz1, pl, Wabt):
        N, dev = pl.N, gz1.device
        g_nb = _empty(dev, N, 128)
        if self.csr_fuse and (self._fuse_mask & 4):
            G_s, G_r = _empty(dev, N, 128), _empty(dev, N, 128)
            ops.rowtile_chain(N, [Seg(gz1, csr=(pl.s_rowptr, pl.s_col), save=G_s), Seg(gz1, csr=(pl.r_rowptr, pl.r_col), save=G_r)],
                              [LayerSpec(Wabt)], [g_nb])
        else:
            G_s = ops.seg_gather_sum(gz1, pl.s_rowptr, pl.s_col, N)
            G_r = ops.seg_gather_sum(gz1, pl.r_rowptr, pl.r_col, N)
            ops.rowtile_chain(N, [Seg(G_s), Seg(G_r)], [LayerSpec(Wabt)], [g_nb])
        return g_nb, G_s, G_r

    def _edge_dw(self, grads, names, M, N, tilesE, G_s, G_r, nb, before=(), after=()):
        lib = L.load()
        dev = grads.flat.device
        tmpE, tmpN = self._edge_tmp(dev)
        layE, layN = [("W1c", "b1", 1), ("W2", "b2", 1), ("W3", "b3", 1)][:len(tilesE)], [("W1ab", None, 2)]
        self._workspace(lib.gfv_dw_multi_workspace_floats(M, len(tilesE), self._layers_block(tmpE, layE)[1])
                        + lib.gfv_dw_multi_workspace_floats(N, 2, self._layers_block(tmpN, layN)[1]) + 8, dev)
        w1, slabs1, blen1, used = self._dw_block(tmpE, layE, tilesE, M, reduce=False)
        w2, slabs2, blen2, _ = self._dw_block(tmpN, layN, [self._tile(G_s, 128, Seg(nb)), self._tile(G_r, 128, Seg(nb))], N,
                                              reduce=False, ws_offset=used)
# ... 382 lines not shown
        st = L.stream_ptr()
        N, E, C = pl.N, pl.E, pl.C
        dev = gloss.device
        gc, gFf = _empty(dev, C, 4), _empty(dev, E, 16)
        gphi, ggrad = _empty(dev, N, 8), _empty(dev, N, 16)
        L.check(lib.gfv_fvm_bwd_ex(sv["cres"].data_ptr(), sv["sums"].data_ptr(), gloss.data_ptr(), sv["Ff"].data_ptr(),
                                pl.cbatch.data_ptr(), pl.theta.data_ptr(), pl.sigma.data_ptr(), pl.dt.data_ptr(),
                                pl.frow.data_ptr(), pl.fk.data_ptr(), pl.kcell.data_ptr(), pl.kS.data_ptr(),
                                pl.ftype.data_ptr(), pl.n_rowptr.data_ptr(), pl.n_col_edge2.data_ptr(), pl.nrow.data_ptr(),
                                pl.ncell.data_ptr(), pl.crow.data_ptr(), pl.pos.data_ptr(), pl.fpos.data_ptr(),
                                pl.centroid.data_ptr(), pl.area.data_ptr(), gc.data_ptr(), gFf.data_ptr(), gphi.data_ptr(),
                                ggrad.data_ptr(), N, E, C, self.nc, None if not self.nc else sv["gradc"].data_ptr(),
                                None if not self.nc else sv["phic"].data_ptr(), st), "fvm_bwd")
        grhs = _empty(dev, N, 8, pl.M)
        L.check(lib.gfv_wlsq_bwd_ex(ggrad.data_ptr(), None, pl.An.data_ptr(), pl.rn.data_ptr(), pl.xo_rowptr.data_ptr(),
                                    pl.xo_in.data_ptr(), pl.xo_B.data_ptr(), pl.sumB.data_ptr(), grhs.data_ptr(),
                                    gphi.data_ptr(), N, pl.M, st), "wlsq_bwd")
        return gphi

    def _normalizer_update(self, src, buffers, N, accumulate, mean_std):
        lib = L.load()
        pws = _empty(src.device, lib.gfv_normalizer_blocks(N), 18)
        sync = accumulate and (self.dist_world > 1 or self.dist_force)
        if sync:
            from . import parallel
            before = parallel.snapshot_normalizer(buffers)

        def update(acc):
            L.check(lib.gfv_normalizer_update(src.data_ptr(), 12, N, 1 if acc else 0, buffers["acc_count"].data_ptr(),
                                              buffers["num_accumulations"].data_ptr(), buffers["acc_sum"].data_ptr(),
                                              buffers["acc_sum_squared"].data_ptr(), pws.data_ptr(),
                                              mean_std.data_ptr(), L.stream_ptr()), "normalizer_update")
        update(accumulate)
        if sync:
            parallel.allreduce_normalizer(buffers, before, self.dist_world, self.dist_group, force=self.dist_force)
            update(False)

    def prep_fwd(self, x, buffers, pl, norm_global, accumulate, want_edge_attr15=True, x_raw=None):
        lib = L.load()
        st = L.stream_ptr()
        N, E, B = pl.N, pl.E, pl.B
        dev = x.device
        assert x.is_contiguous() and x.shape[1] == 12
        if os.environ.get("GFV_PREP_FUSE", "1") == "0" or B > 1024:
            return self._prep_fwd_unfused(x, buffers, pl, norm_global, accumulate, want_edge_attr15, x_raw)
        stats = _empty(dev, B, 6)
        ws = self._prep_ws
        need = lib.gfv_prep_workspace_bytes(B) // 4
        if ws is None or ws.numel() < need or ws.device != dev:
            ws = self._prep_ws = torch.zeros(need, dtype=torch.float32, device=dev)
        mean_std = _empty(dev, 18)
        fused_norm = False
        if norm_global:
            if accumulate:
                self._normalizer_update(x if x_raw is None else x_raw, buffers, N, True, mean_std)
            else:
                fused_norm = True
        own_raw = x_raw is None
        if own_raw:
            x_raw = _empty(dev, N, 12)
        L.check(lib.gfv_prep_stats((x if own_raw else x_raw).data_ptr(), 12, pl.gnode_ptr.data_ptr(), B, stats.data_ptr(), ws.data_ptr(),
                                   x_raw.data_ptr() if own_raw else None,
                                   buffers["acc_count"].data_ptr() if fused_norm else None,
                                   buffers["acc_sum"].data_ptr() if fused_norm else None,
                                   buffers["acc_sum_squared"].data_ptr() if fused_norm else None,
                                   mean_std.data_ptr() if fused_norm else None, st), "prep_stats")
        uv_old = _empty(dev, N, 2)
        ea16 = _empty(dev, E, 16)
        ea15 = _empty(dev, E, 15) if want_edge_attr15 else None
        L.check(lib.gfv_prep_apply(x_raw.data_ptr(), x.data_ptr(), pl.batch.data_ptr(), stats.data_ptr(), pl.uvp_dim.data_ptr(),
                                   mean_std.data_ptr(), 1 if norm_global else 0, uv_old.data_ptr(), N, pl.pos.data_ptr(),
                                   pl.es.data_ptr(), pl.er.data_ptr(), ea16.data_ptr(),
                                   None if ea15 is None else ea15.data_ptr(), E, st), "prep_apply")
        return uv_old, ea16, ea15

    def _prep_fwd_unfused(self, x, buffers, pl, norm_global, accumulate, want_edge_attr15=True, x_raw=None):
        lib = L.load()
        st = L.stream_ptr()
        N, E, B = pl.N, pl.E, pl.B
        dev = x.device
        if x_raw is not None:
            cmdlist.call(x.copy_, x_raw)
        stats = _empty(dev, B, 6)
        nws = _empty(dev, B, 64 * 12)
        L.check(lib.gfv_graph_norm_stats_ws(x.data_ptr(), 12, pl.gnode_ptr.data_ptr(), B, stats.data_ptr(), nws.data_ptr(), st),
                "norm_stats")
        mean_std = _empty(dev, 18)
        if norm_global:
            self._normalizer_update(x, buffers, N, accumulate, mean_std)
        uv_old = _empty(dev, N, 2)
        L.check(lib.gfv_node_prep(x.data_ptr(), 12, pl.batch.data_ptr(), stats.data_ptr(), pl.uvp_dim.data_ptr(),
                                  mean_std.data_ptr(), 1 if norm_global else 0, uv_old.data_ptr(), N, st), "node_prep")
        ea16 = _empty(dev, E, 16)
        ea15 = _empty(dev, E, 15) if want_edge_attr15 else None
        L.check(lib.gfv_edge_attr(x.data_ptr(), 12, pl.pos.data_ptr(), pl.es.data_ptr(), pl.er.data_ptr(), ea16.data_ptr(),
                                  None if ea15 is None else ea15.data_ptr(), E, st), "edge_attr")
        return uv_old, ea16, ea15

    def simulator_fwd(self, P, x, ea16, pl, prefix="simulator", keep=True):
        N, E = pl.N, pl.E
        xn, _, sv_nenc = self.mlp3_fwd(P, f"{prefix}.encoder.nb_encoder", N, [Seg(x, width=12, ld=12)], keep=keep)
        en, _, sv_eenc = self.mlp3_fwd(P, f"{prefix}.encoder.eb_encoder", E, [Seg(ea16, width=15, ld=16)], keep=keep)
        procs = []
        if self.net == "EPD":
            blocks = []
            for ig in range(self.mp):
                xn, en, sv = self.gn_fwd(P, f"{prefix}.GN_block_list.{ig}", xn, en, pl, keep=keep)
                blocks.append(sv)
            procs.append(dict(blocks=blocks, trans=None))
        else:
            pps = [prefix] if self.net == "TransFVGN_v1" else [f"{prefix}.processpr_list.{ip}" for ip in range(self.n_proc)]
            for pp in pps:
                emb = xn
                blocks = []
                for ig in range(self.mp):
                    xn, en, sv = self.gn_fwd(P, f"{pp}.GN_block_list.{ig}", xn, en, pl, keep=keep)
                    blocks.append(sv)
                xn, svt = self.trans_fwd(P, f"{pp}.TransBlock", xn, emb, pl, keep=keep)
                procs.append(dict(blocks=blocks, trans=svt))
        dec, _, sv_dec = self.mlp3_fwd(P, f"{prefix}.decoder.node_decode_module", N, [Seg(xn)], ln=False, keep=keep)
        if not keep:
            return dec, None
        return dec, dict(sv_nenc=sv_nenc, sv_eenc=sv_eenc, procs=procs, sv_dec=sv_dec)

    def simulator_bwd(self, P, sv, g_dec, grads, pl):
        N, E = pl.N, pl.E
        dev = g_dec.device
        g_x = _empty(dev, N, 128)
        self.mlp3_bwd(P, sv["sv_dec"], g_dec, grads, outs=[g_x])
        self.flush()
        g_e = None
        pending = None
        for proc in reversed(sv["procs"]):
            g_emb = None
            if proc["trans"] is not None:
                g_x = self.trans_bwd(P, proc["trans"], g_x, grads, pl, g_add=pending)
                pending = None
                g_emb = g_x
            elif pending is not None:
                g_x, pending = g_x + pending, None
            for blk in reversed(proc["blocks"]):
                if g_e is None:
                    if self._zero_e is None or self._zero_e.shape[0] != E or self._zero_e.device != dev:
                        self._zero_e = torch.zeros((E, 128), dtype=torch.float32, device=dev)
                    g_e = self._zero_e
                self._last_gn = proc is sv["procs"][0] and blk is proc["blocks"][0]
                g_x, g_e = self.gn_bwd(P, blk, g_x, g_e, grads, pl)
            if g_emb is not None:
                pending = g_emb
            if self.bucket_hook is not None and proc is sv["procs"][-1] and len(sv["procs"]) > 1:
                self.flush()
                self.bucket_hook()
        tail = self._tail_cfg(pl)[0] if self._defer_mode else 0
        self.mlp3_bwd(P, sv["sv_eenc"], g_e, grads)
        self.flush(on_main=tail >= 2)
        self.mlp3_bwd(P, sv["sv_nenc"], g_x, grads, g_add=pending)
        self.flush(on_main=tail >= 1)

    def forward(self, P, buffers, x, pl, *, norm_global=True, accumulate=True, want_outputs=True, want_edge_attr15=True,
                before_prep=None, x_raw=None, train_loss=None, keep=True, static_weights=False):
        if static_weights:
            prev = self._wi_static_enter(P)
        else:
            with self.fork():
                prev = self._wi_enter("fwd", P)
        try:
            if before_prep is not None:
                before_prep()
            uv_old, ea16, ea15 = self.prep_fwd(x, buffers, pl, norm_global, accumulate, want_edge_attr15, x_raw=x_raw)
            if not static_weights:
                self.join()
            dec, sv_sim = self.simulator_fwd(P, x, ea16, pl, keep=keep)
        finally:
            if not static_weights:
                self._wi_exit("fwd", prev)
            elif self.f16split:
                ops.set_weight_images(prev)
        if not keep:
            del ea16
        losses, uvp_node, uvp_cell, sv_fvm = self.fvm_fwd(dec, uv_old, pl, want_outputs, train_loss=train_loss, keep=keep)
        return losses, uvp_node, uvp_cell, ea15, (dict(sim=sv_sim, fvm=sv_fvm) if keep else None)

    def backward(self, P, ctx, gloss, grads, pl, g_dec_hook=None):
        with self.fork():
            self.prepare_transposes(P)
            prev = self._wi_enter("bwd", P)
        try:
            g_dec = self.fvm_bwd(ctx["fvm"], gloss, pl)
            if g_dec_hook is not None:
                g_dec_hook(g_dec)
            self.join()
            self.simulator_bwd(P, ctx["sim"], g_dec, grads, pl)
            self.join()
        finally:
            self._wt_live = False
            self._wi_exit("bwd", prev)
        return grads
```

### gen-fvgn-steady_amd/gfv/lib.py

```python
from __future__ import annotations

import ctypes as C
import os

import torch

HERE = os.path.dirname(os.path.abspath(__file__))
LIB_PATH = os.environ.get("GFV_LIB", os.path.join(HERE, "libgfv.so"))

c_float_p = C.c_void_p
c_int_p = C.c_void_p

OP_NONE, OP_BIAS_GELU, OP_MUL_DGELU = 0, 1, 2
IN_NONE, IN_GELU, IN_LN, IN_LNBWD = 0, 1, 2, 3
FIN_PLAIN, FIN_LN, FIN_LNBWD = 0, 1, 2
CHAIN_ROW_OWNER, CHAIN_COLUMN_OWNER = 1, 2
DW_COLSCALE = 8


class Seg(C.Structure):
    _fields_ = [("ptr", C.c_void_p), ("idx", C.c_void_p), ("width", C.c_int32), ("ld", C.c_int32),
                ("csr_rowptr", C.c_void_p), ("csr_scale", C.c_void_p), ("save", C.c_void_p)]


class Layer(C.Structure):
    _fields_ = [("W", C.c_void_p), ("bias", C.c_void_p), ("K", C.c_int32), ("N", C.c_int32), ("op", C.c_int32),
                ("ldw", C.c_int32), ("save", C.c_void_p), ("aux", C.c_void_p), ("Wh", C.c_void_p),
                ("bias2", C.c_void_p)]


class RowtileArgs(C.Structure):
    _fields_ = [
        ("M", C.c_int32), ("nseg", C.c_int32), ("seg", Seg * 3), ("in_add", C.c_void_p), ("in_op", C.c_int32),
        ("nlayers", C.c_int32), ("in_gamma", C.c_void_p), ("in_beta", C.c_void_p), ("in_aux", C.c_void_p),
        ("gadd", C.c_void_p), ("gadd_s", C.c_void_p), ("gadd_r", C.c_void_p), ("in_save", C.c_void_p),
        ("ln_partial", C.c_void_p), ("layer", Layer * 3), ("fin_op", C.c_int32), ("hidden", C.c_int32),
        ("fin_gamma", C.c_void_p), ("fin_beta", C.c_void_p), ("fin_aux", C.c_void_p), ("fin_presave", C.c_void_p),
        ("res", C.c_void_p * 3), ("res_ld", C.c_int32 * 3), ("out_ld", C.c_int32 * 3), ("out", C.c_void_p * 3),
        ("out_nores", C.c_void_p), ("padd", C.c_void_p), ("padd_s", C.c_void_p), ("padd_r", C.c_void_p),
        ("padd_ld", C.c_int32), ("flags", C.c_int32), ("wmax", C.c_void_p),
        ("gscale", C.c_void_p), ("gscale_ld", C.c_int32), ("product_form", C.c_int32),
        ("fin_stats", C.c_void_p), ("in_stats", C.c_void_p), ("dw_partial", C.c_void_p), ("dw_partial_stride", C.c_int64),
        ("dw_in", C.c_void_p), ("dw_in_ld", C.c_int32), ("reserved2_", C.c_int32),
        ("rc_Wh", C.c_void_p * 2), ("rc_bias", C.c_void_p * 2),
    ]


ABI_VERSION = 3

DW_FUSED_FLOATS = 2 * 128 * 128 + 4 * 128
DW_FUSED_WB = 128 * 128 + 128
DW_FUSED_OFF_W3 = 0
DW_FUSED_OFF_W2 = DW_FUSED_WB
DW_FUSED_OFF_LN = 2 * DW_FUSED_WB
assert DW_FUSED_OFF_LN + 256 == DW_FUSED_FLOATS


class WimgDesc(C.Structure):
    _fields_ = [("W", C.c_void_p), ("img", C.c_void_p), ("ldw", C.c_int32), ("N", C.c_int32), ("K", C.c_int32),
                ("reserved", C.c_int32)]


class DwTile(C.Structure):
    _fields_ = [("G", C.c_void_p), ("A", C.c_void_p), ("idx", C.c_void_p), ("in_add", C.c_void_p),
                ("a_gamma", C.c_void_p), ("a_beta", C.c_void_p), ("ldg", C.c_int32), ("n_out", C.c_int32),
                ("width", C.c_int32), ("ld", C.c_int32), ("a_op", C.c_int32), ("ld_out", C.c_int32),
                ("out_off", C.c_int64), ("db_off", C.c_int64), ("gscale", C.c_void_p)]


class ReducePiece(C.Structure):
    _fields_ = [("partial", C.c_void_p), ("out", C.c_void_p), ("chunk_stride", C.c_int64), ("n_chunks", C.c_int32),
                ("rows", C.c_int32), ("cols", C.c_int32), ("ld_in", C.c_int32), ("ld_out", C.c_int32), ("reserved", C.c_int32)]


class TransMlp(C.Structure):
    _fields_ = [("x", C.c_void_p), ("res", C.c_void_p), ("img_out", C.c_void_p), ("img_pre", C.c_void_p), ("img_post", C.c_void_p),
                ("b_out", C.c_void_p), ("b_pre", C.c_void_p), ("b_post", C.c_void_p), ("gamma", C.c_void_p), ("beta", C.c_void_p),
                ("wmax", C.c_void_p), ("fx1", C.c_void_p), ("z", C.c_void_p), ("out", C.c_void_p), ("M", C.c_int32),
                ("reserved", C.c_int32)]


class TransMlpBwd(C.Structure):
    _fields_ = [("g", C.c_void_p), ("g_add", C.c_void_p), ("g_sum", C.c_void_p), ("z", C.c_void_p), ("fx1", C.c_void_p),
                ("img_post_t", C.c_void_p), ("img_pre_t", C.c_void_p), ("img_out_t", C.c_void_p), ("gamma", C.c_void_p),
                ("wmax", C.c_void_p), ("g_z", C.c_void_p), ("g_fx1", C.c_void_p), ("g_out_x", C.c_void_p),
                ("ln_partial", C.c_void_p), ("gscale", C.c_void_p), ("M", C.c_int32), ("reserved", C.c_int32)]


class FvmMesh(C.Structure):
    _fields_ = ([("N", C.c_int32), ("E", C.c_int32), ("C", C.c_int32), ("B", C.c_int32), ("terms", C.c_int32), ("mode", C.c_int32),
                 ("smooth", C.c_int32), ("reserved", C.c_int32)]
                + [(n, C.c_void_p) for n in (
                    "node_type", "batch", "ftype", "cbatch", "gcell_ptr", "pos", "fpos", "y", "centroid", "area", "theta", "sigma",
                    "uvp_dim", "dt", "crow", "kcell", "kS", "frow", "fk", "nfrow", "nfcol2", "nrow", "ncell", "An", "rn",
                    "xo_rowptr", "xo_in", "xo_B", "sumB")])


POOL_MAX_GRAPHS, POOL_MAX_ATTRS, POOL_ROW_HEAD = 64, 56, 8
EVAL_RECORD = 16
TRAIN_LOG_CHUNK, TRAIN_LOG_HEAD, TRAIN_LOG_ENTRY_RECORD, TRAIN_LOG_MAX_BUCKETS = 1024, 16, 8, 32
MARCH_RECORD, MARCH_HEAD, MARCH_GRAPH, MARCH_CONVERGED, MARCH_CAPPED = 16, 8, 8, 1, 2
FIELD_STATS_RECORD, FIELD_STATS_SUMS, FIELD_STATS_AUX = 8, 7, 9
SCHED_RECORD, SCHED_MAX_MILESTONES = 32, 8
SCHED_EVAL, SCHED_TICK, SCHED_FOLLOW = 0, 1, 2
SCHED_STEPEXP, SCHED_EXP, SCHED_GRADUAL, SCHED_TABLE, SCHED_PLATEAU = 1, 2, 3, 4, 5
BALANCE_RECORD, BALANCE_LANES = 32, 64
BALANCE_INVERSE, BALANCE_PROGRESS = 1, 2
OBS_RECORD = 4
POOL_COPY, POOL_ADD, POOL_ROWPTR, POOL_FILL = 0, 1, 2, 3


class PoolArgs(C.Structure):
    _fields_ = [("table_host", C.c_void_p), ("table_dev", C.c_void_p), ("n_entries", C.c_int32), ("n_attrs", C.c_int32),
                ("max_graphs", C.c_int32), ("slice_chunk", C.c_int32), ("max_chunks", C.c_int64),
                ("attr_info", C.c_int32 * POOL_MAX_ATTRS), ("dst", C.c_void_p * POOL_MAX_ATTRS),
                ("dst_cap_words", C.c_int64 * POOL_MAX_ATTRS), ("small", C.c_void_p * 6), ("B", C.c_int32),
                ("reserved", C.c_int32), ("idx", C.c_int32 * POOL_MAX_GRAPHS)]


RENEW_KINDS = {None: 0, "parabolic": 1, "uniform": 2, "uniform_aoa": 3, "Taylor_Green": 4}


class RenewRec(C.Structure):
    _fields_ = [("x", C.c_void_p), ("y", C.c_void_p), ("theta", C.c_void_p), ("dt", C.c_void_p), ("uvp_dim", C.c_void_p),
                ("node_type", C.c_void_p), ("pos", C.c_void_p), ("yrange", C.c_void_p), ("U", C.c_double), ("cos_aoa", C.c_double),
                ("sin_aoa", C.c_double), ("coef", C.c_float * 13), ("N", C.c_int32), ("inlet_kind", C.c_int32),
                ("init_kind", C.c_int32)]


_lib = None

_SIGNATURES = {
    "gfv_pool_renew": (C.c_int, [C.c_void_p, C.c_int32, C.c_void_p]),
    "gfv_pool_args_bytes": (C.c_size_t, []),
    "gfv_pool_table_bytes": (C.c_size_t, [C.c_int32, C.c_int32]),
    "gfv_pool_table_check": (C.c_int, [C.c_void_p, C.c_int32, C.c_int32, C.c_void_p]),
    "gfv_pool_assemble": (C.c_int, [C.POINTER(PoolArgs), C.c_void_p]),
    "gfv_pool_payback": (C.c_int, [C.c_void_p, C.c_void_p, C.c_int32, C.c_int32, C.c_int32, C.c_void_p, C.c_int32, C.c_void_p,
                                   C.c_int64, C.c_void_p, C.c_void_p]),
    "gfv_abi_version": (C.c_int, []),
    "gfv_struct_size": (C.c_int, [C.c_int32]),
    "gfv_seg_gather_sum": (C.c_int, [C.c_void_p, C.c_void_p, C.c_void_p, C.c_void_p, C.c_void_p, C.c_void_p, C.c_int32,
                                     C.c_int32, C.c_int32, C.c_void_p]),
    "gfv_seg_gather_sum_nnz": (C.c_int, [C.c_void_p, C.c_void_p, C.c_void_p, C.c_void_p, C.c_void_p, C.c_void_p, C.c_int32,
                                         C.c_int32, C.c_int32, C.c_int64, C.c_void_p]),
    "gfv_seg_gather_sum_ex": (C.c_int, [C.c_void_p, C.c_void_p, C.c_void_p, C.c_void_p, C.c_void_p, C.c_void_p, C.c_int32,
                                        C.c_int32, C.c_int32, C.c_int64, C.c_int64, C.c_void_p]),
    "gfv_seg_gather_sum_ln": (C.c_int, [C.c_void_p, C.c_void_p, C.c_void_p, C.c_void_p, C.c_void_p, C.c_void_p, C.c_void_p, C.c_int32,
                                        C.c_int64, C.c_int64, C.c_void_p]),
    "gfv_transpose_batch": (C.c_int, [C.c_void_p, C.c_int32, C.c_int32, C.c_int32, C.c_void_p]),
    "gfv_status_flags": (C.c_int, [C.POINTER(C.c_int32)]),
    "gfv_status_mirror": (C.c_int, [C.POINTER(C.POINTER(C.c_int32))]),
    "gfv_status_publish": (C.c_int, [C.c_void_p]),
    "gfv_profile_enable": (C.c_int, [C.c_int]),
    "gfv_profile_collect": (C.c_int, [C.c_int, C.POINTER(C.c_double)]),
    "gfv_profile_reset": (C.c_int, []),
    "gfv_profile_set_sizes": (C.c_int, [C.c_double, C.c_double]),
    "gfv_gather_pair": (C.c_int, [C.c_void_p, C.c_void_p, C.c_void_p, C.c_void_p, C.c_void_p, C.c_int32, C.c_int32,
                                  C.c_void_p]),
    "gfv_get_limit": (C.c_int, [C.c_int32]),
    "gfv_set_limit": (C.c_int, [C.c_int32, C.c_int32]),
    "gfv_limit_name": (C.c_char_p, [C.c_int32]),
    "gfv_rowtile_tiles": (C.c_int, [C.c_int32]),
    "gfv_rowtile_chain": (C.c_int, [C.POINTER(RowtileArgs), C.c_void_p]),
    "gfv_rowtile_last_path": (C.c_int, []),
    "gfv_rowtile_ln_rows": (C.c_int, [C.c_int32]),
    "gfv_rowtile_last_ln_rows": (C.c_int, []),
    "gfv_rowtile_dw_partials": (C.c_int, []),
    "gfv_rowtile_dw_partials_m": (C.c_int, [C.c_int32]),
    "gfv_rowtile_fuses_dw": (C.c_int, [C.POINTER(RowtileArgs)]),
    "gfv_dw_chunks": (C.c_int, [C.c_int32]),
    "gfv_linear_dw_workspace_floats": (C.c_size_t, [C.c_int32, C.c_int32, C.c_int32]),
    "gfv_linear_dw": (C.c_int, [C.c_void_p, C.c_int32, C.c_int32, C.POINTER(Seg), C.c_int32, C.c_void_p, C.c_int32,
                                C.c_int32, C.c_void_p, C.c_void_p, C.c_void_p, C.c_int32, C.c_void_p]),
    "gfv_linear_dw_ex": (C.c_int, [C.c_void_p, C.c_int32, C.c_int32, C.POINTER(Seg), C.c_int32, C.c_void_p, C.c_int32,
                                   C.c_void_p, C.c_void_p, C.c_int32, C.c_void_p, C.c_int32, C.c_void_p, C.c_void_p,
                                   C.c_int32, C.c_void_p]),
    "gfv_linear_dw_gs": (C.c_int, [C.c_void_p, C.c_int32, C.c_int32, C.POINTER(Seg), C.c_int32, C.c_void_p, C.c_int32,
                                   C.c_void_p, C.c_void_p, C.c_int32, C.c_void_p, C.c_void_p, C.c_void_p, C.c_void_p,
                                   C.c_int32, C.c_void_p]),
    "gfv_dw_slabs": (C.c_int, [C.c_int32, C.c_int32, C.c_void_p]),
    "gfv_dw_multi_workspace_floats": (C.c_size_t, [C.c_int32, C.c_int32, C.c_int64]),
    "gfv_dw_multi": (C.c_int, [C.POINTER(DwTile), C.c_int32, C.c_int32, C.c_int64, C.c_void_p, C.c_void_p, C.c_int32,
                               C.c_void_p]),
    "gfv_reduce_partials": (C.c_int, [C.c_void_p, C.c_int32, C.c_int32, C.c_void_p, C.c_int32, C.c_void_p]),
    "gfv_concat_offsets": (C.c_int, [C.c_void_p, C.c_int32, C.c_int32, C.c_void_p]),
    "gfv_f16split_enabled": (C.c_int, []),
    "gfv_set_f16split": (C.c_int, [C.c_int32]),
    "gfv_set_f16split_thread": (C.c_int, [C.c_int32]),
    "gfv_hidden_size": (C.c_int, []),
    "gfv_set_hidden_size": (C.c_int, [C.c_int32]),
    "gfv_weight_image_bytes": (C.c_size_t, [C.c_int32, C.c_int32]),
    "gfv_weight_absmax": (C.c_int, [C.c_void_p, C.c_int32, C.c_void_p, C.c_void_p]),
    "gfv_weight_images": (C.c_int, [C.c_void_p, C.c_int32, C.c_int64, C.c_void_p, C.c_void_p]),
    "gfv_weight_images_form": (C.c_int, [C.c_void_p]),
    "gfv_reduce_partials_2d": (C.c_int, [C.c_void_p, C.c_int32, C.c_int64, C.c_int32, C.c_int32, C.c_int32, C.c_void_p, C.c_void_p]),
    "gfv_reduce_multi": (C.c_int, [C.POINTER(ReducePiece), C.c_int32, C.c_void_p]),
    "gfv_reduce_partials_seg": (C.c_int, [C.c_void_p, C.c_void_p, C.c_int32, C.c_int32, C.c_void_p, C.c_void_p]),
    "gfv_transpose": (C.c_int, [C.c_void_p, C.c_int32, C.c_void_p, C.c_int32, C.c_int32, C.c_void_p]),
    "gfv_slice_softmax_fwd": (C.c_int, [C.c_void_p, C.c_void_p, C.c_void_p, C.c_void_p, C.c_void_p, C.c_int32, C.c_void_p]),
    "gfv_slice_softmax_bwd_blocks": (C.c_int, [C.c_int32]),
    "gfv_slice_softmax_bwd": (C.c_int, [C.c_void_p, C.c_void_p, C.c_void_p, C.c_void_p, C.c_void_p, C.c_void_p, C.c_void_p, C.c_void_p, C.c_int32, C.c_void_p]),
    "gfv_slice_token_partial": (C.c_int, [C.c_void_p, C.c_void_p, C.c_void_p, C.c_void_p, C.c_int32, C.c_void_p, C.c_void_p]),
    "gfv_slice_attention_fwd": (C.c_int, [C.c_void_p, C.c_void_p, C.c_int32, C.c_void_p, C.c_void_p, C.c_void_p, C.c_void_p, C.c_void_p, C.c_void_p, C.c_void_p, C.c_void_p]),
    "gfv_slice_attention_bwd": (C.c_int, [C.c_void_p, C.c_void_p, C.c_int32, C.c_void_p, C.c_void_p, C.c_void_p, C.c_void_p, C.c_void_p, C.c_void_p, C.c_void_p, C.c_void_p, C.c_void_p, C.c_void_p]),
    "gfv_deslice": (C.c_int, [C.c_void_p, C.c_void_p, C.c_void_p, C.c_void_p, C.c_int32, C.c_int32, C.c_void_p]),
    "gfv_slice_gw": (C.c_int, [C.c_void_p, C.c_void_p, C.c_void_p, C.c_void_p, C.c_void_p, C.c_int32, C.c_int32, C.c_void_p]),
    "gfv_slice_softmax_token": (C.c_int, [C.c_void_p] * 7 + [C.c_int32, C.c_void_p, C.c_void_p, C.c_void_p]),
# ... 282 lines not shown
```

### gen-fvgn-steady_amd/gfv/ops.py

```python
from __future__ import annotations

import ctypes as C

import torch

from . import lib as L


def _p(t):
    return None if t is None else t.data_ptr()


def seg_gather_sum(src, rowptr, col, n_rows, scale=None, src_scale=None, out=None, accumulate=False):
    lib = L.load()
    F = src.shape[-1]
    L.f32c(src)
    if out is None:
        assert not accumulate
        out = torch.empty((n_rows, F), dtype=torch.float32, device=src.device)
    rc = lib.gfv_seg_gather_sum_ex(_p(src), _p(L.i32c(rowptr)), _p(L.i32c(col)), _p(scale), _p(src_scale), _p(out),
                                   n_rows, F, 1 if accumulate else 0, col.shape[0], src.shape[0], L.stream_ptr())
    L.check(rc, "gfv_seg_gather_sum")
    return out

# ... 50 lines not shown
        a.ld_in = p.get("ld_in", p["cols"])
        a.ld_out = p.get("ld_out", p["cols"])
    L.check(lib.gfv_reduce_multi(arr, len(pieces), L.stream_ptr()), "gfv_reduce_multi")


def csr_prologue_enabled():
    import os
    return os.environ.get("GFV_CSR_FUSE", "1") != "0"


def rowtile_tiles(M):
    return (M + 63) // 64


def ln_rows(M):
    return (M + 31) // 32


def last_ln_rows():
    return L.load().gfv_rowtile_last_ln_rows()


def gscale_ld(M):
    return (M + 127) // 128 * 8


class Seg:

    def __init__(self, t, idx=None, width=None, ld=None, offset=0, csr=None, scale=None, save=None):
        self.t, self.idx = t, idx
        self.width = t.shape[-1] if width is None else width
        self.ld = t.stride(0) if ld is None else ld
        self.offset = offset
        self.csr, self.scale, self.save = csr, scale, save
        assert csr is None or idx is None

    def fill(self, cs):
        cs.ptr = self.t.data_ptr() + 4 * self.offset
        cs.idx = _p(self.idx) if self.csr is None else self.csr[1].data_ptr()
        cs.width = self.width
        cs.ld = self.ld
        cs.csr_rowptr = None if self.csr is None else self.csr[0].data_ptr()
        cs.csr_scale = _p(self.scale)
        cs.save = _p(self.save)


class LayerSpec:
    def __init__(self, W, bias=None, op=L.OP_NONE, save=None, aux=None, stack=None, bias2=None, stack_cols=None):
        self.W, self.bias, self.op, self.save, self.aux = W, bias, op, save, aux
        self.stack, self.bias2, self.stack_cols = stack, bias2, stack_cols


class WeightImages:

    def __init__(self, device, wmax):
        self.device, self.wmax = device, wmax
        self.images = {}
        self.valid = set()
        self.static = []
        self._desc, self._desc_keys, self._max_frags = None, (), 0
        self._retired = []
        self._bf = None

    def add_static(self, tensors):
        for t in tensors:
            st = t.untyped_storage()
            self.static.append((st.data_ptr(), st.data_ptr() + st.nbytes()))
        self.static.sort()

    def _is_static(self, ptr):
        import bisect
        i = bisect.bisect_right(self.static, (ptr, 1 << 62)) - 1
        return i >= 0 and self.static[i][0] <= ptr < self.static[i][1]

    @staticmethod
    def _parts(key, img):
        if key[0] != "stack":
            return [(key, img.data_ptr())]
        per = img.numel() // (len(key) - 1)
        return [(k, img.data_ptr() + i * per) for i, k in enumerate(key[1:])]

    @staticmethod
    def _upload(items, device):
        parts = [pt for key, img in items for pt in WeightImages._parts(key, img)]
        descs = (L.WimgDesc * len(parts))()
        for d, (key, dst) in zip(descs, parts):
            d.W, d.img, d.ldw, d.N, d.K = key[0], dst, key[1], key[2], key[3]
        return torch.frombuffer(bytearray(bytes(descs)), dtype=torch.uint8).to(device), len(parts)

    def lookup(self, W, stack=None):
        key = (W.data_ptr(), W.stride(0), W.shape[0], W.shape[1])
        if stack is not None:
            assert W.shape == stack.shape and W.shape[0] == 128
            key = ("stack", key, (stack.data_ptr(), stack.stride(0), stack.shape[0], stack.shape[1]))
        bf = L.load().gfv_f16split_enabled() == 3
        if bf != self._bf:
            self._bf = bf
            self.invalidate()
            if self.images and not torch.cuda.is_current_stream_capturing():
                self.build()
        img = self.images.get(key)
        if img is not None:
            return img.data_ptr() if key in self.valid else 0
        blocks = key[1:] if key[0] == "stack" else (key,)
        if not all(self._is_static(k[0]) for k in blocks) or torch.cuda.is_current_stream_capturing():
            return 0
        lib = L.load()
        nbytes = sum(lib.gfv_weight_image_bytes(k[2], k[3]) for k in blocks)
        img = torch.empty((nbytes,), dtype=torch.uint8, device=self.device)
        desc, nd = self._upload([(key, img)], self.device)
        L.check(lib.gfv_weight_images(desc.data_ptr(), nd, img.numel() // 32, self.wmax.data_ptr(), L.stream_ptr()),
                "gfv_weight_images")
        self.images[key] = img
        self.valid.add(key)
        return img.data_ptr()

    def build(self):
        if not self.images:
            return
        if len(self._desc_keys) != len(self.images) and not torch.cuda.is_current_stream_capturing():
            self._desc_keys = tuple(self.images)
            self._retired.append(self._desc)
            self._desc, self._ndesc = self._upload(list(self.images.items()), self.device)
            self._max_frags = max(img.numel() for img in self.images.values()) // 32
        if self._desc is None:
            return
        L.check(L.load().gfv_weight_images(self._desc.data_ptr(), self._ndesc, self._max_frags,
                                           self.wmax.data_ptr(), L.stream_ptr()), "gfv_weight_images")
        self._bf = L.load().gfv_f16split_enabled() == 3
        self.valid = set(self._desc_keys)

    def invalidate(self):
        self.valid = set()


_WI = None


def stack_ready(Wa, Wb, rows=False):
    return (_WI is not None and L.load().gfv_f16split_enabled() and Wa.shape == Wb.shape and Wa.shape[0] == 128
            and _WI.lookup(Wa, Wb) != 0)


def set_weight_images(wi):
    global _WI
    prev, _WI = _WI, wi
    return prev


def rowtile_chain(M, segs, layers, outs, *, in_add=None, in_op=L.IN_NONE, in_gamma=None, in_beta=None, in_aux=None,
                  gadd=None, gadd_s=None, gadd_r=None, in_save=None, ln_partial=None, fin_op=L.FIN_PLAIN,
                  fin_gamma=None, fin_beta=None, fin_aux=None, fin_presave=None, res=None, out_nores=None,
                  padd=None, padd_s=None, padd_r=None, wimg=None, gscale=None, family=0, fin_stats=None, in_stats=None,
                  dw_partial=None, query_fused=False, rc=None):
    lib = L.load()
    wi = wimg if wimg is not None else _WI
    if layers[-1].stack is not None:
        ly = layers[-1]
        h = wi.lookup(ly.W, ly.stack) if (wi is not None and len(layers) == 1 and lib.gfv_f16split_enabled()) else 0
        if not h:
            assert len(layers) == 1 and len(outs) == 2 and res is None and out_nores is None
            kw = dict(in_add=in_add, in_op=in_op, in_gamma=in_gamma, in_beta=in_beta, wimg=wimg)
            rowtile_chain(M, segs, [LayerSpec(ly.W, ly.bias, ly.op)], [outs[0]], in_save=in_save, **kw)
            rowtile_chain(M, segs, [LayerSpec(ly.stack, ly.bias2, ly.op)], [outs[1]], **kw)
            return
    a = L.RowtileArgs()
    a.M = M
    a.nseg = len(segs)
    for i, s in enumerate(segs):
        s.fill(a.seg[i])
    a.in_add = _p(in_add)
    a.in_op = in_op
    a.nlayers = len(layers)
    a.in_gamma, a.in_beta, a.in_aux = _p(in_gamma), _p(in_beta), _p(in_aux)
    a.gadd, a.gadd_s, a.gadd_r = _p(gadd), _p(gadd_s), _p(gadd_r)
    a.in_save, a.ln_partial = _p(in_save), _p(ln_partial)
    for i, ly in enumerate(layers):
        cl = a.layer[i]
        stacked = ly.stack is not None or ly.stack_cols is not None
        cl.W, cl.bias, cl.bias2 = (None if stacked else _p(ly.W)), _p(ly.bias), _p(ly.bias2)
        cl.N = ly.W.shape[0] * (2 if ly.stack is not None else 1)
        cl.K = ly.W.shape[1] * (2 if ly.stack_cols is not None else 1)
        assert ly.W.stride(1) == 1
        cl.ldw = 0 if (ly.stack is not None or ly.stack_cols is not None) else ly.W.stride(0)
        cl.op = ly.op
        cl.save, cl.aux = _p(ly.save), _p(ly.aux)
    if wi is not None:
        hs = [wi.lookup(ly.W, ly.stack if ly.stack is not None else ly.stack_cols) for ly in layers]
        if all(hs):
            for i, h in enumerate(hs):
                a.layer[i].Wh = h
            a.wmax = wi.wmax.data_ptr()
    a.fin_op = fin_op
    a.fin_gamma, a.fin_beta, a.fin_aux, a.fin_presave = _p(fin_gamma), _p(fin_beta), _p(fin_aux), _p(fin_presave)
    for i, o in enumerate(outs):
        t, ld = o if isinstance(o, tuple) else (o, o.stride(0))
        a.out[i] = t.data_ptr() if torch.is_tensor(t) else t
        a.out_ld[i] = ld
    if res is not None:
        for i, o in enumerate(res):
            if o is None:
                continue
            t, ld = o if isinstance(o, tuple) else (o, o.stride(0))
            a.res[i] = t.data_ptr() if torch.is_tensor(t) else t
            a.res_ld[i] = ld
    a.out_nores = _p(out_nores)
    a.flags = family
    a.fin_stats, a.in_stats = _p(fin_stats), _p(in_stats)
    if dw_partial is not None:
        a.dw_partial, a.dw_partial_stride = dw_partial.data_ptr(), dw_partial.stride(0)
    if rc is not None:
        W2, b2, W3, b3 = rc
        h2, h3 = (wi.lookup(W2), wi.lookup(W3)) if wi is not None else (0, 0)
        if not (h2 and h3):
            if query_fused:
                return False
            raise RuntimeError("recompute form: no split-fp16 image of the forward's second / third Linear")
        a.rc_Wh[0], a.rc_Wh[1] = h2, h3
        a.rc_bias[0], a.rc_bias[1] = _p(b2), _p(b3)
    if padd is not None:
        a.padd, a.padd_s, a.padd_r, a.padd_ld = _p(padd), _p(padd_s), _p(padd_r), padd.stride(0)
    if gscale is not None:
        assert gscale.dim() == 2 and gscale.shape[0] >= 3 and gscale.shape[1] >= gscale_ld(M)
        a.gscale, a.gscale_ld = gscale.data_ptr(), gscale.stride(0)
    if query_fused:
        return bool(lib.gfv_rowtile_fuses_dw(C.byref(a)))
    rc = lib.gfv_rowtile_chain(C.byref(a), L.stream_ptr())
    L.check(rc, "gfv_rowtile_chain")
    return gscale is not None and lib.gfv_rowtile_last_path() >= 5


def trans_mlp_fwd(x, res, Wout, bout, gamma, beta, Wpre, bpre, Wpost, bpost, fx1, z, out):
    lib = L.load()
    if _WI is None or not lib.gfv_f16split_enabled():
        return False
    hs = (_WI.lookup(Wout), _WI.lookup(Wpre), _WI.lookup(Wpost))
    if not all(hs):
        return False
    a = L.TransMlp()
    a.x, a.res, a.img_out, a.img_pre, a.img_post = x.data_ptr(), res.data_ptr(), hs[0], hs[1], hs[2]
    a.b_out, a.b_pre, a.b_post = _p(bout), _p(bpre), _p(bpost)
    a.gamma, a.beta, a.wmax = gamma.data_ptr(), beta.data_ptr(), _WI.wmax.data_ptr()
    a.fx1, a.z, a.out, a.M = _p(fx1), _p(z), out.data_ptr(), x.shape[0]
    L.check(lib.gfv_trans_mlp_fwd(C.byref(a), L.stream_ptr()), "gfv_trans_mlp_fwd")
    return True


def trans_mlp_bwd(g, g_add, g_sum, z, fx1, Wpost_t, Wpre_t, Wout_t, gamma, g_z, g_fx1, g_out_x, ln_partial, gscale):
    lib = L.load()
    if _WI is None or not lib.gfv_f16split_enabled():
        return False
    hs = (_WI.lookup(Wpost_t), _WI.lookup(Wpre_t), _WI.lookup(Wout_t))
    if not all(hs):
        return False
    a = L.TransMlpBwd()
    a.g, a.g_add, a.g_sum, a.z, a.fx1 = g.data_ptr(), _p(g_add), _p(g_sum), z.data_ptr(), fx1.data_ptr()
    a.img_post_t, a.img_pre_t, a.img_out_t = hs
    a.gamma, a.wmax = gamma.data_ptr(), _WI.wmax.data_ptr()
    a.g_z, a.g_fx1, a.g_out_x = g_z.data_ptr(), g_fx1.data_ptr(), g_out_x.data_ptr()
    a.ln_partial, a.gscale, a.M = _p(ln_partial), _p(gscale), g.shape[0]
    L.check(lib.gfv_trans_mlp_bwd(C.byref(a), L.stream_ptr()), "gfv_trans_mlp_bwd")
    return True


def linear_dw(G, n_out, segs, M, *, ldg=None, in_add=None, a_op=0, a_gamma=None, a_beta=None, dW=None, db=None,
              want_db=True, accumulate=False, workspace=None, g_offset=0, gscale=None, col_scale=False):
    if col_scale:
        assert a_op == 0
        a_op = L.DW_COLSCALE
    lib = L.load()
    K = sum(s.width for s in segs)
    dev = G.device
    if dW is None:
        dW = torch.empty((n_out, K), dtype=torch.float32, device=dev)
    if db is None and want_db:
        db = torch.empty((n_out,), dtype=torch.float32, device=dev)
    need = lib.gfv_linear_dw_workspace_floats(M, n_out, K)
    if workspace is None or workspace.numel() < need:
        workspace = torch.empty((max(need, 1),), dtype=torch.float32, device=dev)
    cs = (L.Seg * 3)()
    for i, s in enumerate(segs):
        s.fill(cs[i])
    ldg = G.stride(0) if ldg is None else ldg
    rc = lib.gfv_linear_dw_gs(G.data_ptr() + 4 * g_offset, ldg, n_out, cs, len(segs), _p(in_add), a_op, _p(a_gamma),
                              _p(a_beta), M, _p(dW), _p(gscale), _p(db), _p(workspace), 1 if accumulate else 0,
                              L.stream_ptr())
    L.check(rc, "gfv_linear_dw_gs")
    return dW, db
```

### include/gfv.h

```cpp
#ifndef GFV_H_
#define GFV_H_
#include <stddef.h>
#include <stdint.h>

#ifdef __cplusplus
extern "C" {
#endif

#define GFV_ABI_VERSION 3
int gfv_abi_version(void);
int gfv_struct_size(int32_t which);

int gfv_seg_gather_sum(const float* src, const int32_t* rowptr, const int32_t* col, const float* scale,
                       const float* src_scale, float* out, int32_t n_rows, int32_t F, int32_t accumulate, void* stream);

int gfv_seg_gather_sum_nnz(const float* src, const int32_t* rowptr, const int32_t* col, const float* scale,
                           const float* src_scale, float* out, int32_t n_rows, int32_t F, int32_t accumulate,
                           int64_t nnz_hint, void* stream);

int gfv_seg_gather_sum_ex(const float* src, const int32_t* rowptr, const int32_t* col, const float* scale,
                          const float* src_scale, float* out, int32_t n_rows, int32_t F, int32_t accumulate,
                          int64_t nnz_hint, int64_t n_src_hint, void* stream);

int gfv_seg_gather_sum_ln(const float* y, const float* stats, const float* gamma, const float* beta, const int32_t* rowptr,
                          const int32_t* col, float* out, int32_t n_rows, int64_t nnz_hint, int64_t n_src_hint, void* stream);

int gfv_gather_pair(const float* a, const int32_t* s, const int32_t* r, const float* base, float* out,
                    int32_t n_edges, int32_t F, void* stream);

typedef struct {
  const float* ptr;
  const int32_t* idx;
  int32_t width;
  int32_t ld;
  const int32_t* csr_rowptr;
  const float* csr_scale;
  float* save;
} gfv_seg_t;

enum {
  GFV_OP_NONE = 0,
  GFV_OP_BIAS_GELU = 1,
  GFV_OP_MUL_DGELU = 2
};
enum { GFV_IN_NONE = 0, GFV_IN_GELU = 1, GFV_IN_LN = 2, GFV_IN_LNBWD = 3 };
enum { GFV_CHAIN_ROW_OWNER = 1,
       GFV_CHAIN_COLUMN_OWNER = 2    };
enum { GFV_FIN_PLAIN = 0, GFV_FIN_LN = 1, GFV_FIN_LNBWD = 2 };

typedef struct {
  const float* W;
  const float* bias;
  int32_t K, N;
  int32_t op;
  int32_t ldw;
  float* save;
  const float* aux;
  const void* Wh;
  const float* bias2;
} gfv_layer_t;

typedef struct {
  int32_t M;
  int32_t nseg;
  gfv_seg_t seg[3];
  const float* in_add;
  int32_t in_op;
  int32_t nlayers;
  const float* in_gamma;
  const float* in_beta;
  const float* in_aux;
  const float* gadd;
  const int32_t* gadd_s;
  const int32_t* gadd_r;
  float* in_save;
  float* ln_partial;
  gfv_layer_t layer[3];
  int32_t fin_op;
  int32_t hidden;
  const float* fin_gamma;
  const float* fin_beta;
  const float* fin_aux;
  float* fin_presave;
  const float* res[3];
  int32_t res_ld[3];
  int32_t out_ld[3];
  float* out[3];
  float* out_nores;
  const float* padd;
  const int32_t* padd_s;
  const int32_t* padd_r;
  int32_t padd_ld;
  int32_t flags;
  const float* wmax;
  float* gscale;
  int32_t gscale_ld;
  int32_t product_form;
  float* fin_stats;
  const float* in_stats;
  float* dw_partial;
  int64_t dw_partial_stride;
  const float* dw_in;
  int32_t dw_in_ld;
  int32_t reserved2_;
  const void* rc_Wh[2];
  const float* rc_bias[2];
} gfv_rowtile_args_t;
enum { GFV_DW_FUSED_FLOATS = 2 * 128 * 128 + 4 * 128 };
int gfv_rowtile_dw_partials(void);
int gfv_rowtile_dw_partials_m(int32_t M);
int gfv_rowtile_fuses_dw(const gfv_rowtile_args_t* args);

int gfv_rowtile_tiles(int32_t M);
int gfv_rowtile_ln_rows(int32_t M);
int gfv_rowtile_last_ln_rows(void);
int gfv_get_limit(int32_t which);
int gfv_set_limit(int32_t which, int32_t value);
const char* gfv_limit_name(int32_t which);
int gfv_rowtile_chain(const gfv_rowtile_args_t* args, void* stream);
int gfv_rowtile_last_path(void);

typedef struct {
  const float* W;
  void* img;
  int32_t ldw, N, K, reserved;
} gfv_wimg_desc_t;
size_t gfv_weight_image_bytes(int32_t N, int32_t K);
int gfv_f16split_enabled(void);
int gfv_set_f16split(int32_t on);
int gfv_set_f16split_thread(int32_t on);
int gfv_hidden_size(void);
int gfv_set_hidden_size(int32_t h);
int gfv_weight_absmax(const gfv_wimg_desc_t* descs_dev, int32_t n_desc, float* wmax, void* stream);
int gfv_weight_images(const gfv_wimg_desc_t* descs_dev, int32_t n_desc, int64_t max_frags, const float* wmax,
                      void* stream);
int gfv_weight_images_form(const float* wmax);

int gfv_dw_chunks(int32_t M);
int gfv_linear_dw(const float* G, int32_t ldg, int32_t n_out, const gfv_seg_t* segs, int32_t nseg,
                  const float* in_add, int32_t a_gelu, int32_t M, float* dW, float* db, float* workspace,
                  int32_t accumulate, void* stream);
int gfv_linear_dw_gs(const float* G, int32_t ldg, int32_t n_out, const gfv_seg_t* segs, int32_t nseg,
                     const float* in_add, int32_t a_op, const float* a_gamma, const float* a_beta, int32_t M,
                     float* dW, const float* gscale, float* db, float* workspace, int32_t accumulate, void* stream);
size_t gfv_linear_dw_workspace_floats(int32_t M, int32_t n_out, int32_t K);
int gfv_linear_dw_ex(const float* G, int32_t ldg, int32_t n_out, const gfv_seg_t* segs, int32_t nseg,
                     const float* in_add, int32_t a_op, const float* a_gamma, const float* a_beta, int32_t M,
                     float* dW, int32_t reserved, float* db, float* workspace, int32_t accumulate, void* stream);

typedef struct {
  const float* G;
  const float* A;
  const int32_t* idx;
  const float* in_add;
  const float* a_gamma;
  const float* a_beta;
  int32_t ldg, n_out, width, ld;
  int32_t a_op;
  int32_t ld_out;
  int64_t out_off;
  int64_t db_off;
  const float* gscale;
} gfv_dw_tile_t;
enum { GFV_DW_COLSCALE = 8 };
enum { GFV_FLAG_DW_RANGE = 1,
       GFV_FLAG_CHAIN_RANGE = 2 };
int gfv_status_flags(int32_t* flags_out);
int gfv_status_mirror(int32_t** host_word);
int gfv_status_publish(void* stream);
int gfv_dw_slabs(int32_t M, int32_t ntiles, int32_t* rows_per_slab);
size_t gfv_dw_multi_workspace_floats(int32_t M, int32_t ntiles, int64_t block_floats);
int gfv_dw_multi(const gfv_dw_tile_t* tiles, int32_t ntiles, int32_t M, int64_t block_floats, float* workspace,
                 float* grad_block, int32_t accumulate, void* stream);

int gfv_reduce_partials(const float* partial, int32_t n_chunks, int32_t n, float* out, int32_t accumulate,
                        void* stream);

int gfv_reduce_partials_2d(const float* partial, int32_t n_chunks, int64_t chunk_stride, int32_t rows, int32_t cols,
                           int32_t ld_out, float* out, void* stream);

typedef struct {
  const float* partial;
  float* out;
  int64_t chunk_stride;
  int32_t n_chunks, rows, cols, ld_in, ld_out, reserved;
} gfv_reduce_piece_t;
int gfv_reduce_multi(const gfv_reduce_piece_t* pieces, int32_t n_pieces, void* stream);

int gfv_reduce_partials_seg(const float* partial, const int32_t* seg_ptr, int32_t n_seg, int32_t n, float* out,
                            void* stream);

typedef struct {
  const float* in;
  float* out;
  int32_t rows, cols, ld_in, ld_out;
} gfv_transpose_desc_t;
int gfv_transpose_batch(const gfv_transpose_desc_t* descs, int32_t n, int32_t max_rows, int32_t max_cols, void* stream);

typedef struct {
  const void* src;
  void* dst;
  int64_t n_words;
  int32_t kind;
  int32_t add;
} gfv_concat_desc_t;
int gfv_concat_offsets(const gfv_concat_desc_t* descs, int32_t n_desc, int32_t blocks_per_desc, void* stream);

int gfv_transpose(const float* in, int32_t ld_in, float* out, int32_t rows, int32_t cols, void* stream);


int gfv_slice_softmax_fwd(const float* xmid, const float* Ws, const float* bs, const float* temp, float* w, int32_t N,
                          void* stream);
int gfv_slice_softmax_bwd_blocks(int32_t N);
int gfv_slice_softmax_bwd(const float* xmid, const float* Ws, const float* bs, const float* temp, const float* w,
                          const float* gw, float* gxmid, float* partial, int32_t N, void* stream);
int gfv_slice_token_partial(const float* w, const float* a, const int32_t* chunk_beg, const int32_t* chunk_end,
                            int32_t n_chunks, float* partial, void* stream);
int gfv_slice_attention_fwd(const float* partial, const int32_t* gchunk_ptr, int32_t B, const float* Wq, const float* Wk,
                            const float* Wv, float* token, float* norm, float* attn, float* out_token, void* stream);
int gfv_slice_attention_bwd(const float* gpartial, const int32_t* gchunk_ptr, int32_t B, const float* Wq, const float* Wk,
                            const float* Wv, const float* token, const float* norm, const float* attn, float* g_raw,
                            float* g_norm, float* dW_partial, void* stream);
int gfv_slice_softmax_token(const float* xmid, const float* Ws, const float* bs, const float* temp, const float* a,
                            const int32_t* chunk_beg, const int32_t* chunk_end, int32_t n_chunks, float* w, float* partial,
                            void* stream);
int gfv_deslice(const float* w, const float* T, const int32_t* batch, float* out, int32_t N, int32_t accumulate,
                void* stream);
int gfv_slice_gw(const float* a, const float* T, const float* add, const int32_t* batch, float* gw, int32_t N,
                 int32_t accumulate, void* stream);
int gfv_slice_post_bwd(const float* xmid, const float* Ws, const float* bs, const float* temp, const float* w,
                       const float* g_out_x, const float* out_token, const float* fx_mid, const float* g_raw,
                       const float* g_norm, const int32_t* batch, float* g_x_mid, float* g_fx_mid, float* partial,
                       int32_t N, int32_t n_graphs, void* stream);

int gfv_phi_fwd(const float* dec, const float* y, const int32_t* node_type, const float* uv_old, float* phi, int32_t N,
                int32_t mode, void* stream);
int gfv_phi_bwd(const float* gphi, const float* dec, const int32_t* node_type, float* gdec, int32_t N, int32_t mode,
                void* stream);
int gfv_wlsq_fwd(const float* phi, const int32_t* rowptr, const int32_t* outn, const float* Bp, const float* An,
                 const float* rn, float* grad, int32_t N, void* stream);
int gfv_wlsq_bwd(const float* ggrad, const float* An, const float* rn, const int32_t* rowptr_o, const int32_t* inn,
                 const float* Bo, const float* sumB, float* grhs_ws, float* gphi, int32_t N, void* stream);
int gfv_wlsq_fwd_full(const float* phi, const int32_t* rowptr, const int32_t* outn, const float* Bp, const float* An,
                      const float* rn, float* grad, float* full5, int32_t N, void* stream);
int gfv_wlsq_bwd_full(const float* g5, const float* An, const float* rn, const int32_t* rowptr_o, const int32_t* inn,
                      const float* Bo, const float* sumB, float* grhs_ws, float* gphi, int32_t N, void* stream);
int gfv_wlsq_fwd_ex(const float* phi, const int32_t* rowptr, const int32_t* outn, const float* Bp, const float* An,
                    const float* rn, float* grad, float* full, int32_t N, int32_t terms, void* stream);
int gfv_wlsq_bwd_ex(const float* ggrad, const float* gfull, const float* An, const float* rn, const int32_t* rowptr_o,
                    const int32_t* inn, const float* Bo, const float* sumB, float* grhs_ws, float* gphi, int32_t N,
                    int32_t terms, void* stream);
int gfv_face_fwd(const float* phi, const float* grad, const int32_t* es, const int32_t* er, const float* pos,
                 const float* fpos, const int32_t* ftype, const float* y, float* Ff, int32_t E, void* stream);
int gfv_cell_fwd(const float* phi, const float* grad, const float* Ff, const float* pos, const int32_t* crow,
                 const int32_t* kface, const int32_t* knode, const float* kS, const int32_t* ftype, const float* centroid,
                 const float* area, const int32_t* cbatch, const float* theta, const float* dt, const float* uvp_dim,
                 const float* sigma, float* phic, float* cres, float* uvp_cell, int32_t C, void* stream);
int gfv_cell_fwd_ex(const float* phi, const float* grad, const float* Ff, const float* pos, const int32_t* crow,
                    const int32_t* kface, const int32_t* knode, const float* kS, const int32_t* ftype,
                    const float* centroid, const float* area, const int32_t* cbatch, const float* theta, const float* dt,
                    const float* uvp_dim, const float* sigma, float* phic, float* cres, float* uvp_cell, int32_t C,
// ... 335 lines not shown
```

Before: 286.8.

## Fuse narrow first-layer weight gradient into encoder column-chain backward kernel

Extends the fused column-chain backward kernel with a DWN variant for encoder MLPs whose input is narrow (width ≤16). It accumulates the first Linear's weight and bias gradients in LDS with fp32 MFMA instead of writing the gz1 activation gradient to HBM and running a separate GEMM. The encoder edge and node reductions are also merged into a single deferred reduce_multi call. In exchange the kernel uses more LDS and does more per-tile work, which could reduce occupancy.

```diff
diff --git a/gen-fvgn-steady_amd/csrc/colchain.hip b/gen-fvgn-steady_amd/csrc/colchain.hip
--- a/gen-fvgn-steady_amd/csrc/colchain.hip
+++ b/gen-fvgn-steady_amd/csrc/colchain.hip
@@ -27,17 +27,21 @@
   if (a->flags & GFV_CHAIN_ROW_OWNER) return false;
   if (!(a->flags & GFV_CHAIN_COLUMN_OWNER) && (!on || a->M < min_m)) return false;
   if (!a->dw_partial || a->dw_partial_stride < GFV_DW_FUSED_FLOATS || !a->in_stats || !a->wmax) return false;
-  if (a->dw_in) return false;
   const bool noout = a->nlayers == 2;
+  const bool dwn = a->dw_in != nullptr;
+  if (dwn && (!noout || a->dw_in_width < 1 || a->dw_in_width > 16 || a->dw_in_ld < a->dw_in_width ||
+              a->dw_partial_stride < GFV_DW_FUSED_FLOATS_NARROW(a->dw_in_width) || (reinterpret_cast<size_t>(a->dw_in) & 3) ||
+              (size_t)a->M * (size_t)a->dw_in_ld * 4 >= 0x7fffffe0ull))
+    return false;
   const bool rc = a->rc_Wh[0] != nullptr;
-  if (rc && (!a->rc_Wh[1] || a->dw_in || !al16(a->rc_Wh[0]) || !al16(a->rc_Wh[1]) || (a->rc_bias[0] && !al16(a->rc_bias[0])) ||
+  if (rc && (!a->rc_Wh[1] || dwn || !al16(a->rc_Wh[0]) || !al16(a->rc_Wh[1]) || (a->rc_bias[0] && !al16(a->rc_bias[0])) ||
              (a->rc_bias[1] && !al16(a->rc_bias[1]))))
     return false;
   if (!rc && a->rc_Wh[1]) return false;
   if ((a->nlayers != 3 && !noout) || a->in_op != GFV_IN_LNBWD || a->fin_op != GFV_FIN_PLAIN || a->nseg != 1) return false;
-  if (noout && (a->layer[1].op != GFV_OP_MUL_DGELU || a->layer[1].save || a->res[0] || a->gadd || a->dw_in || !a->out[0])) return false;
+  if (noout && (a->layer[1].op != GFV_OP_MUL_DGELU || a->layer[1].save || a->res[0] || a->gadd || (!a->out[0] && !dwn))) return false;
   if (a->seg[0].width != 128 || a->seg[0].idx || a->seg[0].csr_rowptr || a->seg[0].save || a->seg[0].ld != 128 || !al16(a->seg[0].ptr)) return false;
-  if (a->M > (1 << 22) || a->out_ld[0] != 128 || (a->res[0] && a->res_ld[0] != 128) || (a->dw_in && a->dw_in_ld != 128)) return false;
+  if (a->M > (1 << 22) || (a->out_ld[0] != 128 && !dwn) || (a->res[0] && a->res_ld[0] != 128)) return false;
   if (a->layer[0].op != GFV_OP_MUL_DGELU || a->layer[1].op != GFV_OP_MUL_DGELU || (!noout && a->layer[2].op != GFV_OP_NONE)) return false;
   for (int l = 0; l < a->nlayers; ++l) {
     const gfv_layer_t& L = a->layer[l];
@@ -47,10 +51,10 @@
   }
   if ((!rc && (!a->in_aux || !al16(a->in_aux))) || !a->in_gamma || !al16(a->in_gamma) || a->ln_partial || a->padd) return false;
   const bool out2 = !noout && a->layer[2].N == 192;
-  if (!a->out[0] || (out2 ? (!a->out[1] || a->out_ld[1] != 64 || !al16(a->out[1]) || a->dw_in) : a->out[1] != nullptr) || a->out[2] ||
+  if ((!a->out[0] && !dwn) || (out2 ? (!a->out[1] || a->out_ld[1] != 64 || !al16(a->out[1])) : a->out[1] != nullptr) || a->out[2] ||
       a->res[1] || a->res[2] || a->out_nores)
     return false;
-  if ((a->out_ld[0] & 3) || !al16(a->out[0]) || (a->res[0] && ((a->res_ld[0] & 3) || !al16(a->res[0])))) return false;
+  if ((!dwn && ((a->out_ld[0] & 3) || !al16(a->out[0]))) || (a->res[0] && ((a->res_ld[0] & 3) || !al16(a->res[0])))) return false;
   if (a->in_add && !al16(a->in_add)) return false;
   if (a->gadd && (!al16(a->gadd) || !a->gadd_s || !a->gadd_r)) return false;
   if (a->in_save && !al16(a->in_save)) return false;
@@ -79,7 +83,8 @@
 #define CB_K(...) GFV_LAUNCH((colchain_bwd_kernel<__VA_ARGS__>), grid, blk, 0, stream, *a, st)
 #define CB_LAUNCH(LOWP, RC)                                                                                                      \
   do {                                                                                                                           \
-    if (a->nlayers == 2) CB_K(LOWP, false, false, true, RC);                                                                     \
+    if (a->nlayers == 2 && a->dw_in) CB_K(LOWP, false, false, true, false, true);                \
+    else if (a->nlayers == 2) CB_K(LOWP, false, false, true, RC);                                                                \
     else if (a->layer[2].N == 192 && a->gadd) CB_K(LOWP, true, true, false, RC);                                                 \
     else if (a->layer[2].N == 192) CB_K(LOWP, false, true, false, RC);                                                           \
     else if (a->gadd) CB_K(LOWP, true, false, false, RC);                                                                        \
diff --git a/gen-fvgn-steady_amd/csrc/colchain_kernel.h b/gen-fvgn-steady_amd/csrc/colchain_kernel.h
--- a/gen-fvgn-steady_amd/csrc/colchain_kernel.h
+++ b/gen-fvgn-steady_amd/csrc/colchain_kernel.h
@@ -122,7 +122,7 @@
   }
 }
 
-template <bool BF>
+template <bool BF, bool GFRAG = true>
 __device__ __forceinline__ void cb_hidden_bwd(CcCtx& c, int q, const floatx4& acc, float inv_in, const float4& z, float sg,
                                               char* gout, char* aout, float (&v)[4]) {
   const gfv_f2 z01 = {z.x, z.y}, z23 = {z.z, z.w};
@@ -136,7 +136,7 @@
   const float mq = max3_abs(max3_abs(0.f, v[0], v[1]), v[2], v[3]) * sg;
   const float ma = max3_abs(max3_abs(0.f, a[0], a[1]), a[2], a[3]) * (60000.0f / CC_SH_LIMIT);
   c.mabs = fmaxf(c.mabs, q < c.ngt ? fmaxf(mq, ma) : 0.f);
-  cc_put_frag<BF>(gout, q, c, v, sg);
+  if (GFRAG) cc_put_frag<BF>(gout, q, c, v, sg);
   cc_put_frag<BF>(aout, q, c, a, CC_SH);
 }
 
@@ -233,10 +233,11 @@
   }
 }
 
-template <int LOWP, bool GADD, bool OUT2 = false, bool NOOUT = false, bool RC = false>
+template <int LOWP, bool GADD, bool OUT2 = false, bool NOOUT = false, bool RC = false, bool DWN = false>
 __global__ __launch_bounds__(64 * CC_W, 2) void colchain_bwd_kernel(const gfv_rowtile_args_t A, int* status) {
+  static_assert(!DWN || (NOOUT && !RC), "the narrow first-layer weight gradient exists in the plain NOOUT forms only");
   constexpr int TG = CB_TG;
-  __shared__ __attribute__((aligned(16))) char lds[CbLds::TOTAL + (RC ? CbLds::BUF : 0)];
+  __shared__ __attribute__((aligned(16))) char lds[CbLds::TOTAL + (RC ? CbLds::BUF : DWN ? 64 * CC_W * 20 : 0)];
   char* b0 = lds + CbLds::B0;
   char* b1 = lds + CbLds::B1;
   char* b2 = lds + CbLds::B2;
@@ -268,7 +269,7 @@
   B.z1 = cb_buf(A.layer[1].aux, rows128);
   B.gadd = cb_buf(A.gadd, 0x7fffffe0ull);
   B.gidx = cb_buf(c.w < 4 ? A.gadd_s : A.gadd_r, (size_t)A.M * 4);
-  B.save1 = cb_buf(NOOUT ? A.out[0] : A.layer[1].save, rows128);
+  B.save1 = cb_buf(DWN ? nullptr : NOOUT ? A.out[0] : A.layer[1].save, rows128);
   B.res = cb_buf(NOOUT ? nullptr : A.res[0], rows128);
   B.out = cb_buf(NOOUT ? nullptr : A.out[0], rows128);
   const cb_rsrc out2 = cb_buf(OUT2 ? A.out[1] : nullptr, (size_t)A.M * 256);
@@ -281,6 +282,14 @@
 #pragma unroll
   for (int kt = 0; kt < 8; ++kt) dw3[kt] = dw2[kt] = floatx4{0.f, 0.f, 0.f, 0.f};
   float dgam[4] = {0.f, 0.f, 0.f, 0.f}, dbet[4] = {0.f, 0.f, 0.f, 0.f};
+  constexpr int DW1_OFF = CbLds::TOTAL, DB1_OFF = DW1_OFF + 64 * CC_W * 16;
+#define CB_PK reinterpret_cast<float*>(b0 + c.w * 4096)
+#define CB_DW1P (reinterpret_cast<floatx4*>(lds + DW1_OFF) + (c.w * 64 + c.lane))
+#define CB_DB1P (reinterpret_cast<float*>(lds + DB1_OFF) + (c.w * 64 + c.lane))
+  if constexpr (DWN) {
+    *CB_DW1P = floatx4{0.f, 0.f, 0.f, 0.f};
+    *CB_DB1P = 0.f;
+  }
   float sacc = 0.f;
   float scap = 3.0e38f;
 
@@ -582,6 +591,16 @@
     CT(6);
     cc_barrier();
     CT(7);
+    float xb[DWN ? 4 * TG : 1];
+    if constexpr (DWN) {
+      const cb_rsrc xr = cb_buf(A.dw_in, ((size_t)(A.M - 1) * A.dw_in_ld + A.dw_in_width) * 4);
+      const int rlim = c.j < A.dw_in_width ? min(c.M, c.row0 + 16 * c.ngt) : 0;
+      const int xo = (c.row0 + c.g) * (A.dw_in_ld * 4) + c.j * 4;
+#pragma unroll
+      for (int i = 0; i < 4 * TG; ++i)
+        xb[i] = __builtin_bit_cast(float, __builtin_amdgcn_raw_buffer_load_b32(
+                                              xr, c.row0 + c.g + 4 * i < rlim ? xo + 4 * i * (A.dw_in_ld * 4) : CB_OFF_DEAD, 0, 0));
+    }
     {
       const float inv_in = 1.0f / s2s;
       floatx4 a0, a1;
@@ -599,11 +618,17 @@
           cb_hidden_bwd_dg<LOWP == 2>(c, 2 * p, a0, inv_in, d0, s1s, b0, v0);
           cb_hidden_bwd_dg<LOWP == 2>(c, 2 * p + 1, a1, inv_in, d1, s1s, b0, v1);
         } else {
-          cb_hidden_bwd<LOWP == 2>(c, 2 * p, a0, inv_in, zq[2 * p], s1s, b0, b2, v0);
-          cb_hidden_bwd<LOWP == 2>(c, 2 * p + 1, a1, inv_in, zq[2 * p + 1], s1s, b0, b2, v1);
-        }
-        cb_st4(B.save1, offS[2 * p], v0);
-        cb_st4(B.save1, offS[2 * p + 1], v1);
+          cb_hidden_bwd<LOWP == 2, !DWN>(c, 2 * p, a0, inv_in, zq[2 * p], s1s, b0, b2, v0);
+          cb_hidden_bwd<LOWP == 2, !DWN>(c, 2 * p + 1, a1, inv_in, zq[2 * p + 1], s1s, b0, b2, v1);
+        }
+        if constexpr (DWN) {
+          float* d = CB_PK + (2 * p) * 256 + c.j * 16 + 4 * c.g;
+          *reinterpret_cast<float4*>(d) = make_float4(v0[0], v0[1], v0[2], v0[3]);
+          *reinterpret_cast<float4*>(d + 256) = make_float4(v1[0], v1[1], v1[2], v1[3]);
+        } else {
+          cb_st4(B.save1, offS[2 * p], v0);
+          cb_st4(B.save1, offS[2 * p + 1], v1);
+        }
         if (CB_LATE && p + 1 < TG / 2) cc_mma_pair<4, LOWP, true>(b1, p + 1, wh, wl, c.lane, n0, n1);
         a0 = n0; a1 = n1;
       }
@@ -669,6 +694,22 @@
         cb_load_inputs(B, c, next_row0, in);
         cb_load_gathers<GADD>(B, c, gidx, in);
       }
+      if constexpr (DWN) {
+        floatx4 dw1 = *CB_DW1P;
+        float db1 = *CB_DB1P;
+#pragma unroll
+        for (int q = 0; q < TG; ++q) {
+          if (q >= c.ngt) break;
+#pragma unroll
+          for (int s = 0; s < 4; ++s) {
+            const float gv = CB_PK[q * 256 + s * 64 + c.lane];
+            db1 += gv;
+            dw1 = __builtin_amdgcn_mfma_f32_16x16x4f32(gv, xb[4 * q + s], dw1, 0, 0, 0);
+          }
+        }
+        *CB_DW1P = dw1;
+        *CB_DB1P = db1;
+      }
       cb_dw_tile<LOWP>(b1, b2, np, c.w, c.lane, dw2, db2);
     }
     CT(11);
@@ -682,6 +723,8 @@
 #endif
   if (A.dw_partial) {
     float* blk = A.dw_partial + (size_t)blockIdx.x * A.dw_partial_stride;
+    const int elane = DWN ? (int)__builtin_amdgcn_mbcnt_hi(~0u, __builtin_amdgcn_mbcnt_lo(~0u, 0u)) : c.lane;
+    const int ej = DWN ? (elane & 15) : c.j, eg = DWN ? (elane >> 4) : c.g, ecol0 = DWN ? 16 * c.w + 4 * eg : c.col0;
     const float is = sacc != 0.f ? 1.0f / sacc : 0.f;
     const float r2 = 1.0f / step1, r1 = r2 / step2;
     const float u3 = is * CC_SH_INV, u2 = (is * r2) * CC_SH_INV;
@@ -689,14 +732,14 @@
     for (int kt = 0; kt < 8; ++kt)
 #pragma unroll
       for (int r = 0; r < 4; ++r) {
-        const int n = 16 * cb_dw_ntile(c.w, kt) + 4 * c.g + r, k = 16 * cb_dw_ktile(c.w, kt) + c.j;
+        const int n = 16 * cb_dw_ntile(c.w, kt) + 4 * eg + r, k = 16 * cb_dw_ktile(c.w, kt) + ej;
         blk[n * 128 + k] = dw3[kt][r] * u3;
         blk[16384 + 128 + n * 128 + k] = dw2[kt][r] * u2;
       }
-    if (c.j == 0) {
+    if (ej == 0) {
 #pragma unroll
       for (int r = 0; r < 4; ++r) {
-        const int nb = 16 * cb_dw_btile(c.w) + 4 * c.g + r;
+        const int nb = 16 * cb_dw_btile(c.w) + 4 * eg + r;
         blk[16384 + nb] = db3[r] * is;
         blk[2 * 16384 + 128 + nb] = db2[r] * (is * r2);
       }
@@ -704,14 +747,30 @@
 #pragma unroll
     for (int r = 0; r < 4; ++r) {
       const float dg = gfv_row16_sum(dgam[r]), db = gfv_row16_sum(dbet[r]);
-      if (c.j == 0) {
-        blk[2 * 16384 + 256 + c.col0 + r] = dg;
-        blk[2 * 16384 + 384 + c.col0 + r] = db;
-      }
+      if (ej == 0) {
+        blk[2 * 16384 + 256 + ecol0 + r] = dg;
+        blk[2 * 16384 + 384 + ecol0 + r] = db;
+      }
+    }
+    if constexpr (DWN) {
+      const int width = A.dw_in_width;
+      float* blk1 = blk + GFV_DW_FUSED_FLOATS;
+      const floatx4 dw1 = *CB_DW1P;
+      const float db1 = *CB_DB1P;
+      if (ej < width) {
+#pragma unroll
+        for (int r = 0; r < 4; ++r) blk1[(ecol0 + r) * width + ej] = dw1[r];
+      }
+      const float s01 = db1 + __shfl_xor(db1, 16, 64);
+      const float sb = s01 + __shfl_xor(s01, 32, 64);
+      if (eg == 0) blk1[128 * width + 16 * c.w + ej] = sb;
     }
   }
   if (c.mabs > 60000.0f) atomicOr(status, 2);
-}
-
-
-}
+#undef CB_PK
+#undef CB_DW1P
+#undef CB_DB1P
+}
+
+
+}
diff --git a/gen-fvgn-steady_amd/csrc/rowtile.hip b/gen-fvgn-steady_amd/csrc/rowtile.hip
--- a/gen-fvgn-steady_amd/csrc/rowtile.hip
+++ b/gen-fvgn-steady_amd/csrc/rowtile.hip
@@ -216,6 +216,10 @@
       const int nfused = 2 + (args->rc_Wh[0] ? 2 : 0);
       fl += nfused * 2.0 * args->M * 128.0 * 128.0;
       by += 8.0 * args->M + 4.0 * (double)gfv_rowtile_dw_partials_m(args->M) * (double)args->dw_partial_stride;
+      if (args->dw_in) {
+        fl += 2.0 * args->M * 128.0 * (double)args->dw_in_width;
+        by += 4.0 * args->M * ((double)args->dw_in_width - (double)last.N);
+      }
     }
     tok = gfv_prof_begin(kind, fl, by, (hipStream_t)stream);
   }
diff --git a/gen-fvgn-steady_amd/gfv/engine.py b/gen-fvgn-steady_amd/gfv/engine.py
--- a/gen-fvgn-steady_amd/gfv/engine.py
+++ b/gen-fvgn-steady_amd/gfv/engine.py
@@ -121,6 +121,8 @@
         self._tail_main = int(os.environ.get("GFV_TAIL_MAIN", "2"))
         self._tail_split = int(os.environ.get("GFV_TAIL_SPLIT", "1"))
         self._fuse_noout = os.environ.get("GFV_FUSE_NOOUT", "1") != "0"
+        self._fuse_narrow_dw1 = os.environ.get("GFV_FUSE_NARROW_DW1", "1") != "0"
+        self._enc_reduce_merge = os.environ.get("GFV_ENC_REDUCE_MERGE", "1") != "0"
         self._fuse_dw_min = int(os.environ.get("GFV_COLCHAIN_BWD_MIN_M", "2048"))
         self._cbwd_max_fixed = None
         self._wi, self._wi_key, self._wmax, self._wi_abs = None, None, None, None
@@ -399,7 +401,7 @@
         ops.rowtile_chain(M, [Seg(sv["z1"])], [LayerSpec(P[names[2]], P[names[3]], L.OP_BIAS_GELU, save=sv["z2"]),
                                               LayerSpec(P[names[4]], P[names[5]])], [sv["y3"]], in_op=L.IN_GELU)
 
-    def mlp3_bwd(self, P, sv, G, grads, *, outs=None, res=None, gadd=None, W1t=None, g_ld=None, g_add=None):
+    def mlp3_bwd(self, P, sv, G, grads, *, outs=None, res=None, gadd=None, W1t=None, g_ld=None, g_add=None, collect=None):
         prefix, M, ln = sv["prefix"], sv["M"], sv["ln"]
         names = self._mlp_names(prefix, ln)
         W1, W2, W3 = P[names[0]], P[names[2]], P[names[4]]
@@ -409,7 +411,8 @@
         if (self.fuse_dw and ln and sv.get("fused", sv.get("stats") is not None) and G.stride(0) == 128 and g_ld is None and gadd is None
                 and (outs is not None or (res is None and self._fuse_noout))
                 and self._mlp3_bwd_fused(P, sv, G, grads, names, W3t, W2t,
-                                         None if outs is None else (W1t if W1t is not None else self._T(W1)), outs, res, g_add)):
+                                         None if outs is None else (W1t if W1t is not None else self._T(W1)), outs, res, g_add,
+                                         collect)):
             return
         self._rematerialize(P, sv)
         gz2, gz1 = _empty(dev, M, 128), _empty(dev, M, 128)
@@ -452,10 +455,37 @@
         self.defer(side, gz1, gz2, g3, G, part, gs, sv["z1"], sv["z2"], sv["in_add"], *[sg.t for sg in sv["segs"]],
                    *[sg.idx for sg in sv["segs"]])
 
-    def _mlp3_bwd_fused(self, P, sv, G, grads, names, W3t, W2t, W1t, outs, res, g_add):
+    def _mlp3_bwd_fused_narrow(self, P, sv, G, grads, names, W3t, W2t, g_add, collect):
+        M, sg = sv["M"], sv["segs"][0]
+        width = sg.width
+        nwg = L.load().gfv_rowtile_dw_partials_m(M)
+        FL = L.dw_fused_floats_narrow(width)
+        dwp = _empty(G.device, nwg, FL)
+        layers = [LayerSpec(W3t, None, L.OP_MUL_DGELU, aux=sv["z2"]), LayerSpec(W2t, None, L.OP_MUL_DGELU, aux=sv["z1"])]
+        kw = dict(in_op=L.IN_LNBWD, in_gamma=P[names[6]], in_aux=sv["y3"], in_stats=sv["stats"], dw_partial=dwp, in_add=g_add,
+                  dw_in=(sg.t.data_ptr() + 4 * sg.offset, width, sg.ld))
+        if not ops.rowtile_chain(M, [Seg(G)], layers, [None], query_fused=True, **kw):
+            return False
+        ops.rowtile_chain(M, [Seg(G)], layers, [None], **kw)
+        first = self._gview2(grads, names[0], names[1])
+        assert first.numel() == 128 * (width + 1)
+        pieces = self._fused_pieces(dwp, nwg, grads, names, FL)
+        pieces.append(self._piece(dwp.data_ptr() + 4 * L.DW_FUSED_FLOATS, first, nwg, FL, 128 * (width + 1)))
+        if collect is not None:
+            collect.append((pieces, (dwp, sg.t)))
+        else:
+            self.defer(lambda: ops.reduce_multi(pieces), dwp, sg.t)
+        return True
+
+    def _mlp3_bwd_fused(self, P, sv, G, grads, names, W3t, W2t, W1t, outs, res, g_add, collect=None):
         M = sv["M"]
         dev = G.device
         lib = L.load()
+        if (outs is None and res is None and self._fuse_narrow_dw1 and sv["z2"] is not None and sv["in_add"] is None
+                and len(sv["segs"]) == 1 and sv["segs"][0].width <= 16 and sv["segs"][0].idx is None and sv["segs"][0].csr is None
+                and P[names[0]].shape[1] == sv["segs"][0].width
+                and self._mlp3_bwd_fused_narrow(P, sv, G, grads, names, W3t, W2t, g_add, collect)):
+            return True
         nwg = lib.gfv_rowtile_dw_partials_m(M)
         dwp = _empty(dev, nwg, L.DW_FUSED_FLOATS)
         gz1 = _empty(dev, M, 128)
@@ -496,8 +526,8 @@
     def _ln_piece(self, part, n_rows, grads, gamma, beta):
         return self._piece(part, self._gview2(grads, gamma, beta), n_rows, 256, 256)
 
-    def _fused_pieces(self, dwp, nwg, grads, names):
-        base, FL, WB = dwp.data_ptr(), L.DW_FUSED_FLOATS, L.DW_FUSED_WB
+    def _fused_pieces(self, dwp, nwg, grads, names, FL=L.DW_FUSED_FLOATS):
+        base, WB = dwp.data_ptr(), L.DW_FUSED_WB
         return [self._piece(base + 4 * L.DW_FUSED_OFF_W2, self._gview2(grads, names[2], names[3]), nwg, FL, WB),
                 self._piece(base + 4 * L.DW_FUSED_OFF_W3, self._gview2(grads, names[4], names[5]), nwg, FL, WB),
                 self._piece(base + 4 * L.DW_FUSED_OFF_LN, self._gview2(grads, names[6], names[7]), nwg, FL, 256)]
@@ -1186,9 +1216,13 @@
                 self.flush()
                 self.bucket_hook()
         tail = self._tail_cfg(pl)[0] if self._defer_mode else 0
-        self.mlp3_bwd(P, sv["sv_eenc"], g_e, grads)
+        enc = [] if self._enc_reduce_merge else None
+        self.mlp3_bwd(P, sv["sv_eenc"], g_e, grads, collect=enc)
         self.flush(on_main=tail >= 2)
-        self.mlp3_bwd(P, sv["sv_nenc"], g_x, grads, g_add=pending)
+        self.mlp3_bwd(P, sv["sv_nenc"], g_x, grads, g_add=pending, collect=enc)
+        if enc:
+            pieces = [p for ps, _ in enc for p in ps]
+            self.defer(lambda: ops.reduce_multi(pieces), *[t for _, keep in enc for t in keep])
         self.flush(on_main=tail >= 1)
 
     def forward(self, P, buffers, x, pl, *, norm_global=True, accumulate=True, want_outputs=True, want_edge_attr15=True,
diff --git a/gen-fvgn-steady_amd/gfv/lib.py b/gen-fvgn-steady_amd/gfv/lib.py
--- a/gen-fvgn-steady_amd/gfv/lib.py
+++ b/gen-fvgn-steady_amd/gfv/lib.py
@@ -41,7 +41,7 @@
         ("padd_ld", C.c_int32), ("flags", C.c_int32), ("wmax", C.c_void_p),
         ("gscale", C.c_void_p), ("gscale_ld", C.c_int32), ("product_form", C.c_int32),
         ("fin_stats", C.c_void_p), ("in_stats", C.c_void_p), ("dw_partial", C.c_void_p), ("dw_partial_stride", C.c_int64),
-        ("dw_in", C.c_void_p), ("dw_in_ld", C.c_int32), ("reserved2_", C.c_int32),
+        ("dw_in", C.c_void_p), ("dw_in_ld", C.c_int32), ("dw_in_width", C.c_int32),
         ("rc_Wh", C.c_void_p * 2), ("rc_bias", C.c_void_p * 2),
     ]
 
@@ -54,6 +54,10 @@
 DW_FUSED_OFF_W2 = DW_FUSED_WB
 DW_FUSED_OFF_LN = 2 * DW_FUSED_WB
 assert DW_FUSED_OFF_LN + 256 == DW_FUSED_FLOATS
+
+
+def dw_fused_floats_narrow(width):
+    return DW_FUSED_FLOATS + 128 * (width + 1)
 
 
 class WimgDesc(C.Structure):
diff --git a/gen-fvgn-steady_amd/gfv/ops.py b/gen-fvgn-steady_amd/gfv/ops.py
--- a/gen-fvgn-steady_amd/gfv/ops.py
+++ b/gen-fvgn-steady_amd/gfv/ops.py
@@ -226,7 +226,7 @@
                   gadd=None, gadd_s=None, gadd_r=None, in_save=None, ln_partial=None, fin_op=L.FIN_PLAIN,
                   fin_gamma=None, fin_beta=None, fin_aux=None, fin_presave=None, res=None, out_nores=None,
                   padd=None, padd_s=None, padd_r=None, wimg=None, gscale=None, family=0, fin_stats=None, in_stats=None,
-                  dw_partial=None, query_fused=False, rc=None):
+                  dw_partial=None, query_fused=False, rc=None, dw_in=None):
     lib = L.load()
     wi = wimg if wimg is not None else _WI
     if layers[-1].stack is not None:
@@ -268,6 +268,8 @@
     a.fin_op = fin_op
     a.fin_gamma, a.fin_beta, a.fin_aux, a.fin_presave = _p(fin_gamma), _p(fin_beta), _p(fin_aux), _p(fin_presave)
     for i, o in enumerate(outs):
+        if o is None:
+            continue
         t, ld = o if isinstance(o, tuple) else (o, o.stride(0))
         a.out[i] = t.data_ptr() if torch.is_tensor(t) else t
         a.out_ld[i] = ld
@@ -283,6 +285,9 @@
     a.fin_stats, a.in_stats = _p(fin_stats), _p(in_stats)
     if dw_partial is not None:
         a.dw_partial, a.dw_partial_stride = dw_partial.data_ptr(), dw_partial.stride(0)
+    if dw_in is not None:
+        t, width, ld = dw_in
+        a.dw_in, a.dw_in_width, a.dw_in_ld = (t.data_ptr() if torch.is_tensor(t) else t), width, ld
     if rc is not None:
         W2, b2, W3, b3 = rc
         h2, h3 = (wi.lookup(W2), wi.lookup(W3)) if wi is not None else (0, 0)
diff --git a/include/gfv.h b/include/gfv.h
--- a/include/gfv.h
+++ b/include/gfv.h
@@ -102,11 +102,13 @@
   int64_t dw_partial_stride;
   const float* dw_in;
   int32_t dw_in_ld;
-  int32_t reserved2_;
+  int32_t dw_in_width;
   const void* rc_Wh[2];
   const float* rc_bias[2];
 } gfv_rowtile_args_t;
 enum { GFV_DW_FUSED_FLOATS = 2 * 128 * 128 + 4 * 128 };
+#define GFV_DW_FUSED_FLOATS_NARROW(width) (GFV_DW_FUSED_FLOATS + 128 * ((width) + 1))
+enum { GFV_DW_FUSED_FLOATS_NARROW_MAX = GFV_DW_FUSED_FLOATS + 128 * 17 };
 int gfv_rowtile_dw_partials(void);
 int gfv_rowtile_dw_partials_m(int32_t M);
 int gfv_rowtile_fuses_dw(const gfv_rowtile_args_t* args);
```

After: 287.5, median of 2. Within noise of the previous version (+0.2%).
